# shgaurav1/DVG

Measured on AMD Instinct MI355X. Metric: predicted frames/sec at 64x64, batch 64, 10-in/10-out, higher is better.
Workload: dtype f32

## Files before the change

dvg_amd/csrc/conv_igemm2.hip:

```cpp
#include <cstdlib>
#include <type_traits>

#include "dvg_common.h"

namespace dvg {

constexpr int DVG_GEMM_WGS_PER_CU = DVG_BF16X3 ? 3 : 4;
constexpr int DVG_GEMM128_WGS = DVG_BF16X3 ? 3 : 2;
constexpr int DVG_GEMM128_GT = DVG_BF16X3 ? 2 : 4;
constexpr int DVG_GEMM_GT = 4;
constexpr int DVG_GEMM128_MIN_WGS = 4 * 768;
[[maybe_unused]] constexpr int DVG_GEMM_NT2 = 256;
constexpr int DVG_TILE16_MIN_WGS = 256;

enum { M2_CONV3 = 0, M2_CONV4S2 = 1, M2_CONVT4S2 = 2, M2_GEMM = 3 };

struct Igemm2Params {
    const float* x = nullptr;
    const float* skip = nullptr;
    const float* w = nullptr;
    const float* scale = nullptr;
    const float* shift = nullptr;
    float* y = nullptr;
    float* y_pool = nullptr;
// ... 1007 lines not shown
    const int a_base = (wm * 32 + l31) * LD + hh * 4;
    const int b_base = (wn * 32 + l31) * LDB + (hh ^ ((l31 >> 3) & 1)) * 4;

    f32x16 acc[4];
#pragma unroll
    for (int f = 0; f < 4; ++f)
#pragma unroll
        for (int i = 0; i < 16; ++i) acc[f][i] = 0.f;

    long offx[FIRST ? 1 : ND];
    unsigned okmask = 0;
#pragma unroll
    for (int i = 0; i < ND; ++i) {
        const int hp = (tid + i * 256) >> 2;
        const int yy = yin0 + hp / C::HW, xx = xin0 + hp % C::HW;
        const bool ok = hp < C::HP && (unsigned)yy < (unsigned)p.H && (unsigned)xx < (unsigned)p.W;
        okmask |= ok ? (1u << i) : 0u;
        if constexpr (!FIRST) offx[i] = ok ? (((long)n0 * p.H + yy) * p.W + xx) * p.C1 + (tid & 3) * 4 : 0;
    }
    const int xf = (tid >> 2) & 3, xq = tid & 3;
    const int x_ia = xf == 0 ? 0 : (xf == 2 ? 2 : 1), x_ib = xf == 2 ? 1 : (xf == 3 ? 3 : 2);
    const float x_sg = xf == 1 ? 1.f : -1.f;
    const int x_pix = (tid >> 7) * C::HW + 2 * ((tid >> 4) & 7);
    const int x_da = (x_pix + x_ia) * 16 + xq * 4, x_db = (x_pix + x_ib) * 16 + xq * 4;
    const int x_st = xf * C::PLANE + (tid >> 4) * LD + (xq >> 1) * 4 + (xq & 1) * 2;

    f32x4 fw[FIRST ? 11 : 1];
    f32x4 ra[ND], rb[NLB];
    auto gload_d = [&](int c0) {
        if constexpr (FIRST) {
            const float* w = p.first_w + c0 + (tid & 3) * 4;
#pragma unroll
            for (int tp = 0; tp < 9; ++tp) fw[tp] = *reinterpret_cast<const f32x4*>(w + tp * 64);
            fw[9] = *reinterpret_cast<const f32x4*>(p.first_scale + c0 + (tid & 3) * 4);
            fw[10] = *reinterpret_cast<const f32x4*>(p.first_shift + c0 + (tid & 3) * 4);
        } else {
            const float* src = p.x + c0;
#pragma unroll
            for (int i = 0; i < ND; ++i)
                ra[i] = *reinterpret_cast<const f32x4*>(((okmask >> i) & 1u) ? src + offx[i] : dvg_zero_slot);
        }
    };
    auto store_d = [&]() {
        if constexpr (FIRST) {
#pragma unroll
            for (int i = 0; i < ND; ++i) {
                const int hp = min((tid + i * 256) >> 2, C::HP - 1);
                const float* f = Fp + (hp / C::HW) * C::FP_W + hp % C::HW;
                f32x4 v = {0.f, 0.f, 0.f, 0.f};
#pragma unroll
                for (int tp = 0; tp < 9; ++tp) {
                    const float px = f[(tp / 3) * C::FP_W + tp % 3];
#pragma unroll
                    for (int e = 0; e < 4; ++e) v[e] = fmaf(fw[tp][e], px, v[e]);
                }
                const float okf = (float)((okmask >> i) & 1u);
#pragma unroll
                for (int e = 0; e < 4; ++e) {
                    const float a = v[e] * fw[9][e] + fw[10][e];
                    v[e] = fmaxf(a, a * p.first_slope) * okf;
                }
                ra[i] = v;
            }
        }
#pragma unroll
        for (int i = 0; i < ND; ++i) reinterpret_cast<f32x4*>(Ds)[tid + i * 256] = ra[i];
    };
    auto gload_b = [&](int chunk, int r) {
        const float* tile = p.w + (((size_t)chunk * (p.Cout >> 6) + nb) * 12 + r * 4) * (64 * C::WROW);
#pragma unroll
        for (int j = 0; j < NLB; ++j) rb[j] = reinterpret_cast<const f32x4*>(tile)[tid + j * 256];
    };
    auto store_b = [&]() {
#pragma unroll
        for (int j = 0; j < NLB; ++j) reinterpret_cast<f32x4*>(Bs)[tid + j * 256] = rb[j];
    };
    auto xform_read = [&](u32x2_t (&pa)[NX][3]) {
#pragma unroll
        for (int s = 0; s < NX; ++s) {
            const f32x4 a = *reinterpret_cast<const f32x4*>(&Ds[x_da + s * 2 * C::HW * 16]);
            const f32x4 b = *reinterpret_cast<const f32x4*>(&Ds[x_db + s * 2 * C::HW * 16]);
            f32x4 v;
#pragma unroll
            for (int e = 0; e < 4; ++e) v[e] = fmaf(x_sg, b[e], a[e]);
            unsigned t0, t1, t2;
            bf16x3_split_pair(v[0], v[1], t0, t1, t2);
            pa[s][0][0] = t0; pa[s][1][0] = t1; pa[s][2][0] = t2;
            bf16x3_split_pair(v[2], v[3], t0, t1, t2);
            pa[s][0][1] = t0; pa[s][1][1] = t1; pa[s][2][1] = t2;
        }
    };
    auto xform_store = [&](const u32x2_t (&pa)[NX][3]) {
#pragma unroll
        for (int s = 0; s < NX; ++s)
#pragma unroll
            for (int j = 0; j < 3; ++j) *reinterpret_cast<u32x2_t*>(&As[x_st + s * 16 * LD + j * 8]) = pa[s][j];
    };

    if constexpr (FIRST) {
        const float* fr = p.first_frame + (size_t)n0 * p.H * p.W;
        for (int i = tid; i < C::FP_FLOATS; i += 256) {
            const int yy = yin0 - 1 + i / C::FP_W, xx = xin0 - 1 + i % C::FP_W;
            Fp[i] = ((unsigned)yy < (unsigned)p.H && (unsigned)xx < (unsigned)p.W) ? fr[(size_t)yy * p.W + xx] : 0.f;
        }
        __syncthreads();
    }
    gload_d(0);
    gload_b(0, 0);
    store_d();
    store_b();
    __syncthreads();
    {
        u32x2_t pa[NX][3];
        xform_read(pa);
        xform_store(pa);
    }
    __syncthreads();

    auto stage = [&](const int chunk, auto r_c, auto next_chunk_c, auto has_next_c) __attribute__((always_inline)) {
        constexpr int R = decltype(r_c)::value;
        constexpr bool NEXT_CHUNK = decltype(next_chunk_c)::value, HAS_NEXT = decltype(has_next_c)::value;
        constexpr bool LOAD_D = NEXT_CHUNK && R == 0, STORE_D = NEXT_CHUNK && R == 1, XFORM = NEXT_CHUNK && R == 2;
        if constexpr (LOAD_D) gload_d((chunk + 1) * 16);
        if constexpr (HAS_NEXT) gload_b(R == 2 ? chunk + 1 : chunk, (R + 1) % 3);
        if constexpr (STORE_D) store_d();
        u32x2_t pa[XFORM ? NX : 1][3];
        if constexpr (XFORM) xform_read(pa);

        f32x4 fa[2][3], fb[2][3];
#pragma unroll
        for (int j = 0; j < 3; ++j) {
            fa[0][j] = *reinterpret_cast<const f32x4*>(&As[a_base + R * C::TP * LD + j * 8]);
            fb[0][j] = *reinterpret_cast<const f32x4*>(&Bs[b_base + j * 8]);
        }
#pragma unroll
        for (int tt = 0; tt < 4; ++tt) {
            const int cur = tt & 1, nxt = cur ^ 1;
            if (tt + 1 < 4) {
#pragma unroll
                for (int j = 0; j < 3; ++j) {
                    fa[nxt][j] = *reinterpret_cast<const f32x4*>(&As[a_base + (tt + 1) * C::PLANE + R * C::TP * LD + j * 8]);
                    fb[nxt][j] = *reinterpret_cast<const f32x4*>(&Bs[b_base + (tt + 1) * 64 * LDB + j * 8]);
                }
            }
            if (HAS_NEXT && tt == 3) {
                __syncthreads();
                if constexpr (XFORM) xform_store(pa);
                store_b();
            }
            auto mm = [&](int pa_, int pb_) {
                acc[tt] = __builtin_amdgcn_mfma_f32_32x32x16_bf16(__builtin_bit_cast(bf16x8_t, fa[cur][pa_]),
                                                                  __builtin_bit_cast(bf16x8_t, fb[cur][pb_]), acc[tt], 0, 0, 0);
            };
            mm(2, 0);
            mm(1, 1);
            mm(0, 2);
            mm(1, 0);
            mm(0, 1);
            mm(0, 0);
            constexpr int NREAD = 6, NMFMA = 6;
            constexpr int NVMEM = (LOAD_D ? (FIRST ? 11 : ND) : 0) + (HAS_NEXT ? NLB : 0), VPT = (NVMEM + 2) / 3;
            if (tt == 0) __builtin_amdgcn_sched_group_barrier(0x100, NREAD + (XFORM ? 2 * NX : 0) + (STORE_D && FIRST ? 9 * ND : 0), 0);
            if (tt + 1 < 4) {
#pragma unroll
                for (int r = 0; r < NREAD; ++r) {
                    __builtin_amdgcn_sched_group_barrier(0x100, 1, 0);
                    __builtin_amdgcn_sched_group_barrier(0x008, 1, 0);
                }
                if (VPT > 0) __builtin_amdgcn_sched_group_barrier(0x020, VPT, 0);
            } else if (HAS_NEXT) {
                constexpr int NW = NLB + (XFORM ? 3 * NX : 0);
#pragma unroll
                for (int r = 0; r < NW; ++r) {
                    if (r < NMFMA) __builtin_amdgcn_sched_group_barrier(0x008, 1, 0);
                    __builtin_amdgcn_sched_group_barrier(0x200, 1, 0);
                }
            } else if (!HAS_NEXT) {
                __builtin_amdgcn_sched_group_barrier(0x008, NMFMA, 0);
            }
        }
        if constexpr (HAS_NEXT) __syncthreads();
    };
    using std::integral_constant;
    using T_ = integral_constant<bool, true>;
    using F_ = integral_constant<bool, false>;
    int st = 0;
    auto set_prio = [&]() {
        switch (st++ & 3) {
            case 0: __builtin_amdgcn_s_setprio(3); break;
            case 1: __builtin_amdgcn_s_setprio(2); break;
            case 2: __builtin_amdgcn_s_setprio(1); break;
            default: __builtin_amdgcn_s_setprio(0); break;
        }
    };
    const int nchunks = p.C1 / 16;
    int chunk = 0;
    for (; chunk + 1 < nchunks; ++chunk) {
        set_prio();
        stage(chunk, integral_constant<int, 0>{}, T_{}, T_{});
        set_prio();
        stage(chunk, integral_constant<int, 1>{}, T_{}, T_{});
        set_prio();
        stage(chunk, integral_constant<int, 2>{}, T_{}, T_{});
    }
    set_prio();
    stage(chunk, integral_constant<int, 0>{}, F_{}, T_{});
    set_prio();
    stage(chunk, integral_constant<int, 1>{}, F_{}, T_{});
    set_prio();
    stage(chunk, integral_constant<int, 2>{}, F_{}, F_{});
    __builtin_amdgcn_s_setprio(0);

    const int c = nb0 + wn * 32 + l31;
    const float sc = p.scale ? p.scale[c] : 1.f, sf = p.shift ? p.shift[c] : 0.f;
    const bool want_y = !FIRST || n0 >= p.y_from;
    float* const yb = p.y + (size_t)n0 * p.H * p.W * p.Cout + c;
    float* const pb = p.y_pool ? p.y_pool + (size_t)n0 * (p.H >> 1) * (p.W >> 1) * p.Cout + c : nullptr;
    const float* ab = nullptr;
    if (p.addend) ab = p.addend + (size_t)(addend_image(p.add_map, p.add_B, n0)) * p.H * p.W * p.Cout + c;
    auto epilogue = [&](auto act_c) {
        constexpr int ACT = decltype(act_c)::value;
        float v[2][16];
#pragma unroll
        for (int reg = 0; reg < 16; ++reg) {
            v[0][reg] = (acc[0][reg] + acc[1][reg]) + acc[2][reg];
            v[1][reg] = (acc[1][reg] - acc[2][reg]) - acc[3][reg];
        }
#pragma unroll
        for (int reg = 0; reg < 16; ++reg) {
            const int m = wm * 32 + (reg & 3) + 8 * (reg >> 2) + 4 * hh;
            const int off = ((y0 + (m >> 3)) * p.W + x0 + 2 * (m & 7)) * p.Cout;
#pragma unroll
            for (int e = 0; e < 2; ++e) {
                float u = v[e][reg];
                if (ab != nullptr) u += ab[off + e * p.Cout];
                u = u * sc + sf;
                if constexpr (ACT == DVG_ACT_LRELU) u = u > 0.f ? u : u * p.slope;
                else if constexpr (ACT != DVG_ACT_NONE) u = apply_act(u, p.act, p.slope);
                v[e][reg] = u;
                if (want_y) yb[off + e * p.Cout] = u;
            }
        }
        if (pb != nullptr) {
#pragma unroll
            for (int reg = 0; reg < 16; ++reg) {
                if (((reg >> 2) & 1) == 0) {
                    const int m = wm * 32 + (reg & 3) + 8 * (reg >> 2) + 4 * hh;
                    const float mx = fmaxf(fmaxf(v[0][reg], v[1][reg]), fmaxf(v[0][reg + 4], v[1][reg + 4]));
                    pb[(((y0 + (m >> 3)) >> 1) * (p.W >> 1) + (x0 >> 1) + (m & 7)) * p.Cout] = mx;
                }
            }
        }
    };
    if (p.act == DVG_ACT_LRELU) epilogue(std::integral_constant<int, DVG_ACT_LRELU>{});
    else if (p.act == DVG_ACT_NONE) epilogue(std::integral_constant<int, DVG_ACT_NONE>{});
    else epilogue(std::integral_constant<int, -1>{});
}

template <bool FIRST>
static int launch_wx(Igemm2Params p, hipStream_t stream) {
    using C = CfgWX;
    p.tiles_y = p.H / C::TH;
    p.tiles_x = p.W / C::TW;
    p.tiles_n = p.N;
    p.nblk_n = p.Cout / 64;
    const long tiles = (long)p.tiles_y * p.tiles_x * p.tiles_n;
    p.nb_group = choose_nb_group(tiles, p.nblk_n, 12.0 * p.C1 * 64 * 4, (double)C::TH * C::TW * p.C1 * 4);
    static bool attr_set = false;
    if (!attr_set) {
        hipError_t e = hipFuncSetAttribute(reinterpret_cast<const void*>(&conv3_wx_kernel<FIRST>),
                                           hipFuncAttributeMaxDynamicSharedMemorySize, C::lds_bytes(FIRST));
        if (e != hipSuccess) return fail(DVG_ERR_HIP, "hipFuncSetAttribute: %s", hipGetErrorString(e));
        attr_set = true;
    }
    hipLaunchKernelGGL((conv3_wx_kernel<FIRST>), dim3((unsigned)(tiles * p.nblk_n)), dim3(256), C::lds_bytes(FIRST), stream, p);
    return check_launch("conv3_wx");
}
#endif

__global__ void pack_wx_kernel(const float* __restrict__ src, float* __restrict__ dst, int cout, int cin) {
    const long total = (long)cout * cin * 12 / 2;
    const int nblk = cout >> 6;
    for (long i = blockIdx.x * (long)blockDim.x + threadIdx.x; i < total; i += (long)gridDim.x * blockDim.x) {
        const int k = (int)(i & 7) * 2;
        long r = i >> 3;
        const int co = r % cout; r /= cout;
        const int tap = r % 12;
        const int chunk = r / 12;
        const int row = tap >> 2, f = tap & 3;
        float u[2];
#pragma unroll
        for (int e = 0; e < 2; ++e) {
            const float* g = src + (((long)co * cin + chunk * 16 + k + e) * 3 + row) * 3;
            if (f == 0) u[e] = g[0];
            else if (f == 1) u[e] = ((g[0] + g[1]) + g[2]) * 0.5f;
            else if (f == 2) u[e] = ((g[0] - g[1]) + g[2]) * 0.5f;
            else u[e] = g[2];
        }
        wrow_store_pair(dst, (((size_t)chunk * nblk + (co >> 6)) * 12 + tap) * 64 + (co & 63), co & 63, k, u[0], u[1]);
    }
    wrow_drain();
}

__global__ void pack_k16_kernel(const float* __restrict__ src, float* __restrict__ dst, int cout, int cin, int kh,
                                int kw, int transposed) {
    const long total = (long)cout * cin * kh * kw / 2;
    const int nblk = cout >> 6, taps = kh * kw;
    for (long i = blockIdx.x * (long)blockDim.x + threadIdx.x; i < total; i += (long)gridDim.x * blockDim.x) {
        const int k = (int)(i & 7) * 2;
        long r = i >> 3;
        const int co = r % cout; r /= cout;
        const int t = r % taps;
        const int chunk = r / taps;
        const int ci = chunk * 16 + k, a = t / kw, b = t % kw;
        const long j = transposed ? ((((long)ci * cout + co) * kh + (kh - 1 - a)) * kw + (kw - 1 - b))
                                  : ((((long)co * cin + ci) * kh + a) * kw + b);
        const long j1 = j + (transposed ? (long)cout * kh * kw : (long)kh * kw);
        int slot = t;
        if (transposed && kh == 4 && kw == 4) {
            const int py = a & 1, px = b & 1;
            slot = (py * 2 + px) * 4 + ((2 + py - a) >> 1) * 2 + ((2 + px - b) >> 1);
        } else if (kh == 4 && kw == 4) {
            slot = ((a & 1) * 2 + (b & 1)) * 4 + (a >> 1) * 2 + (b >> 1);
        }
        wrow_store_pair(dst, (((size_t)chunk * nblk + (co >> 6)) * taps + slot) * 64 + (co & 63), co & 63, k, src[j], src[j1]);
    }
    wrow_drain();
}

}

using namespace dvg;

extern "C" int dvg_mfma_mode(void) { return DVG_BF16X3 ? 1 : 0; }
extern "C" int dvg_packed_row_floats(void) { return DVG_WROW; }

extern "C" void dvg_debug_set_clockbuf(void* buf, unsigned records) {
    g_clk = (unsigned long long*)buf;
    g_clk_cap = buf ? records : 0;
}

extern "C" int dvg_pack_conv_weight_k16(const float* w, float* w_packed, int cout, int cin, int kh, int kw,
                                        int transposed, void* stream) {
    DVG_REQUIRE(w && w_packed, DVG_ERR_NULL, "dvg_pack_conv_weight_k16: NULL pointer");
    DVG_REQUIRE(cout > 0 && cout % 64 == 0 && cin > 0 && cin % 16 == 0 && kh > 0 && kw > 0, DVG_ERR_SHAPE,
                "dvg_pack_conv_weight_k16: Cin must be a multiple of 16, Cout of 64");
    const long total = (long)cout * cin * kh * kw / 2;
    long g = (total + 255) / 256;
    if (g > 4096) g = 4096;
    hipLaunchKernelGGL(pack_k16_kernel, dim3((unsigned)g), dim3(256), 0, (hipStream_t)stream, w, w_packed, cout, cin, kh,
                       kw, transposed);
    return check_launch("dvg_pack_conv_weight_k16");
}

extern "C" int dvg_conv_splitk_v2(int mode, int N, int H, int W, int Cin, int Cout) {
    Plan2 pl;
    if (Cin % 16 || Cout % 64 || plan2(&pl, mode, N, H, W, Cin, Cout, true, false)) return -1;
    return pl.splitk;
}

extern "C" int dvg_conv_stats_rows_v2(int mode, int N, int H, int W, int Cin, int Cout, int pool, int with_workspace) {
    Plan2 pl;
    if (plan2(&pl, mode, N, H, W, Cin, Cout, with_workspace != 0, pool != 0)) return -1;
    return pl.stats_rows;
}

static Igemm2Params params2(const float* x, const float* skip, const float* w, const float* scale, const float* shift, float* y,
                            int N, int H, int W, int C1, int C2, int Cout, int act, float slope) {
    Igemm2Params p{};
    p.x = x; p.skip = skip; p.w = w; p.scale = scale; p.shift = shift; p.y = y;
    p.N = N; p.H = H; p.W = W; p.C1 = C1; p.C2 = C2; p.Cout = Cout;
    p.act = act; p.slope = slope;
    return p;
}

static int set_addend(Igemm2Params& p, const char* who, const float* addend, const int* addend_map, int addend_block) {
    p.addend = addend;
    p.add_map = addend ? addend_map : nullptr;
    p.add_B = addend_block;
    DVG_REQUIRE(p.add_map == nullptr || (addend_block > 0 && p.N % addend_block == 0), DVG_ERR_SHAPE,
                "%s: addend_block must divide N", who);
    return DVG_OK;
}

static int checks2(const Igemm2Params& p, const char* who) {
    DVG_REQUIRE(p.x && p.w && p.y, DVG_ERR_NULL, "%s: x/w/y must not be NULL", who);
    DVG_REQUIRE((p.skip != nullptr) == (p.C2 > 0), DVG_ERR_SHAPE, "%s: skip pointer / C2 mismatch", who);
    DVG_REQUIRE(p.N > 0 && p.H > 0 && p.W > 0, DVG_ERR_SHAPE, "%s: empty shape", who);
    DVG_REQUIRE(p.C1 > 0 && p.C1 % 16 == 0 && p.C2 % 16 == 0, DVG_ERR_SHAPE, "%s: C1=%d C2=%d must be multiples of 16",
                who, p.C1, p.C2);
    DVG_REQUIRE(p.Cout > 0 && p.Cout % 64 == 0, DVG_ERR_SHAPE, "%s: Cout=%d must be a multiple of 64", who, p.Cout);
    DVG_REQUIRE(aligned16(p.x) && aligned16(p.w) && aligned16(p.y) && aligned16(p.skip), DVG_ERR_ALIGN,
                "%s: pointers must be 16-byte aligned", who);
    DVG_REQUIRE(p.act >= DVG_ACT_NONE && p.act <= DVG_ACT_SIGMOID, DVG_ERR_SHAPE, "%s: bad act", who);
    return DVG_OK;
}

extern "C" int dvg_conv3x3_bn_act_v2(const float* x, const float* skip, const float* w_k16, const float* scale,
                                     const float* shift, float* y, float* y_pool, float* stats, int N, int H, int W,
                                     int C1, int C2, int Cout, int upsample_x, int act, float slope,
                                     float* workspace, long workspace_floats, const float* addend,
                                     const int* addend_map, int addend_block, void* stream) {
    const char* who = "dvg_conv3x3_bn_act_v2";
    Igemm2Params p = params2(x, skip, w_k16, scale, shift, y, N, H, W, C1, C2, Cout, act, slope);
    p.y_pool = y_pool;
    p.stats = stats;
    p.upsample = upsample_x ? 1 : 0;
    if (int e = set_addend(p, who, addend, addend_map, addend_block)) return e;
    if (int e = checks2(p, who)) return e;
    DVG_REQUIRE(aligned16(addend) && (addend == nullptr || y_pool == nullptr), DVG_ERR_SHAPE,
                "%s: addend must be 16-byte aligned and excludes the pooled output", who);
    DVG_REQUIRE(H % 8 == 0 && W % 8 == 0, DVG_ERR_SHAPE, "%s: H=%d W=%d must be multiples of 8", who, H, W);
    Plan2 pl;
    DVG_REQUIRE(plan2(&pl, M2_CONV3, N, H, W, C1 + C2, Cout, workspace != nullptr, y_pool != nullptr) == 0 && pl.ti == 1,
                DVG_ERR_SHAPE, "%s: no tile for %dx%d", who, H, W);
    return launch_tile<M2_CONV3>(p, pl, who, workspace, workspace_floats, stream);
}

static int first_pair_params(Igemm2Params* out, const char* who, const float* frame, const float* w0, const float* scale0,
                             const float* shift0, const float* w1, const float* scale1, const float* shift1, float* y,
                             float* y_pool, int N, int H, int W, int Cout, int act, float slope, int y_from) {
    DVG_REQUIRE(y_from >= 0 && y_from <= N && (y_from == 0 || y_pool != nullptr) && (y != nullptr || y_from == N), DVG_ERR_SHAPE,
                "%s: y_from=%d needs 0 <= y_from <= N, a pooled output when > 0, y unless == N", who, y_from);
    float* const y_biased = y ? y - (size_t)y_from * H * W * Cout : y_pool;
    Igemm2Params p = params2(frame , nullptr, w1, scale1, shift1, y_biased, N, H, W, 64, 0, Cout,
                             act, slope);
    p.y_pool = y_pool;
    p.first_frame = frame; p.first_w = w0; p.first_scale = scale0; p.first_shift = shift0; p.first_slope = 0.2f;
    p.y_from = y_from;
    *out = p;
    return DVG_OK;
}

extern "C" int dvg_conv3x3_first_pair(const float* frame, const float* w0, const float* scale0, const float* shift0,
                                      const float* w1_k16, const float* scale1, const float* shift1, float* y, float* y_pool,
                                      int N, int H, int W, int Cout, int act, float slope, int y_from, void* stream) {
    const char* who = "dvg_conv3x3_first_pair";
    DVG_REQUIRE(frame && w0 && scale0 && shift0, DVG_ERR_NULL, "%s: NULL pointer", who);
    Igemm2Params p;
    if (int e = first_pair_params(&p, who, frame, w0, scale0, shift0, w1_k16, scale1, shift1, y, y_pool, N, H, W, Cout, act, slope,
                                  y_from))
        return e;
    if (int e = checks2(p, who)) return e;
    DVG_REQUIRE(H % 8 == 0 && W % 16 == 0 && (long)N * (H / 8) * (W / 16) * (Cout / 64) >= 512, DVG_ERR_SHAPE,
                "%s: H %% 8, W %% 16 and >= 512 workgroups needed (N=%d H=%d W=%d Cout=%d)", who, N, H, W, Cout);
    Plan2 pl;
    if (plan2(&pl, M2_CONV3, N, H, W, 64, Cout, false, y_pool != nullptr, true)) return fail(DVG_ERR_SHAPE, "%s: no tile", who);
    return launch2<M2_CONV3, Tile2<1, 8, 16>, true>(p, pl, nullptr, 0, (hipStream_t)stream);
}

extern "C" int dvg_pack_conv_weight_wx(const float* w, float* w_packed, int cout, int cin, void* stream) {
    DVG_REQUIRE(w && w_packed, DVG_ERR_NULL, "dvg_pack_conv_weight_wx: NULL pointer");
    DVG_REQUIRE(cout > 0 && cout % 64 == 0 && cin > 0 && cin % 16 == 0, DVG_ERR_SHAPE,
                "dvg_pack_conv_weight_wx: Cin must be a multiple of 16, Cout of 64");
    DVG_REQUIRE(aligned16(w_packed), DVG_ERR_ALIGN, "dvg_pack_conv_weight_wx: w_packed must be 16-byte aligned");
    const long total = (long)cout * cin * 12 / 2;
    hipLaunchKernelGGL(pack_wx_kernel, dim3(grid_for(total, 256, 4096)), dim3(256), 0, (hipStream_t)stream, w, w_packed, cout, cin);
    return check_launch("dvg_pack_conv_weight_wx");
}

static int checks_wx(const Igemm2Params& p, const char* who) {
    DVG_REQUIRE(p.N > 0 && p.H > 0 && p.W > 0, DVG_ERR_SHAPE, "%s: empty shape", who);
    DVG_REQUIRE(p.C1 > 0 && p.C1 % 16 == 0 && p.C2 == 0 && p.skip == nullptr && !p.upsample, DVG_ERR_SHAPE,
                "%s: Cin=%d must be a multiple of 16; no concat operand, no upsampling", who, p.C1 + p.C2);
    DVG_REQUIRE(p.Cout > 0 && p.Cout % 64 == 0, DVG_ERR_SHAPE, "%s: Cout=%d must be a multiple of 64", who, p.Cout);
    DVG_REQUIRE(p.H % 8 == 0 && p.W % 16 == 0, DVG_ERR_SHAPE, "%s: H=%d must be a multiple of 8, W=%d of 16", who, p.H, p.W);
    DVG_REQUIRE((long)p.H * p.W * p.Cout < (1L << 31), DVG_ERR_SHAPE, "%s: image of %d x %d x %d floats too large", who, p.H, p.W, p.Cout);
    DVG_REQUIRE(aligned16(p.x) && aligned16(p.w) && aligned16(p.y) && aligned16(p.y_pool) && aligned16(p.addend), DVG_ERR_ALIGN,
                "%s: pointers must be 16-byte aligned", who);
    DVG_REQUIRE(p.act >= DVG_ACT_NONE && p.act <= DVG_ACT_SIGMOID, DVG_ERR_SHAPE, "%s: bad act", who);
    DVG_REQUIRE(DVG_BF16X3 != 0, DVG_ERR_SHAPE, "%s: the f32-MFMA build has no WX kernel", who);
    return DVG_OK;
}

extern "C" int dvg_conv3x3_bn_act_wx(const float* x, const float* skip, const float* w_wx, const float* scale,
                                     const float* shift, float* y, float* y_pool, int N, int H, int W, int C1, int C2,
                                     int Cout, int upsample_x, int act, float slope, const float* addend,
                                     const int* addend_map, int addend_block, void* stream) {
    const char* who = "dvg_conv3x3_bn_act_wx";
    DVG_REQUIRE(x && w_wx && y, DVG_ERR_NULL, "%s: x/w/y must not be NULL", who);
    Igemm2Params p = params2(x, skip, w_wx, scale, shift, y, N, H, W, C1, C2, Cout, act, slope);
    p.y_pool = y_pool;
    p.upsample = upsample_x ? 1 : 0;
    if (int e = set_addend(p, who, addend, addend_map, addend_block)) return e;
    DVG_REQUIRE(addend == nullptr || y_pool == nullptr, DVG_ERR_SHAPE, "%s: addend excludes the pooled output", who);
    if (int e = checks_wx(p, who)) return e;
#if DVG_BF16X3
    return launch_wx<false>(p, (hipStream_t)stream);
#else
    return DVG_ERR_SHAPE;
#endif
}

extern "C" int dvg_conv3x3_first_pair_wx(const float* frame, const float* w0, const float* scale0, const float* shift0,
                                         const float* w1_wx, const float* scale1, const float* shift1, float* y, float* y_pool,
                                         int N, int H, int W, int Cout, int act, float slope, int y_from, void* stream) {
    const char* who = "dvg_conv3x3_first_pair_wx";
    DVG_REQUIRE(frame && w0 && scale0 && shift0 && w1_wx, DVG_ERR_NULL, "%s: NULL pointer", who);
    Igemm2Params p;
    if (int e = first_pair_params(&p, who, frame, w0, scale0, shift0, w1_wx, scale1, shift1, y, y_pool, N, H, W, Cout, act, slope,
                                  y_from))
        return e;
    DVG_REQUIRE(aligned16(w0) && aligned16(scale0) && aligned16(shift0) && aligned16(y), DVG_ERR_ALIGN,
                "%s: pointers must be 16-byte aligned", who);
    if (int e = checks_wx(p, who)) return e;
#if DVG_BF16X3
    return launch_wx<true>(p, (hipStream_t)stream);
#else
    return DVG_ERR_SHAPE;
#endif
}

extern "C" int dvg_conv4x4s2_bn_act_v2(const float* x, const float* w_k16, const float* scale, const float* shift,
                                       float* y, float* stats, int N, int H, int W, int Cin, int Cout, int act,
                                       float slope, float* workspace, long workspace_floats, void* stream) {
    const char* who = "dvg_conv4x4s2_bn_act_v2";
    Igemm2Params p = params2(x, nullptr, w_k16, scale, shift, y, N, H, W, Cin, 0, Cout, act, slope);
    p.stats = stats;
    if (int e = checks2(p, who)) return e;
    DVG_REQUIRE(H % 2 == 0 && W % 2 == 0, DVG_ERR_SHAPE, "%s: odd input", who);
    DVG_REQUIRE((long)N * H * W * Cin < (1L << 31), DVG_ERR_SHAPE,
                "%s: input of %d x %d x %d x %d floats too large (32-bit offsets)", who, N, H, W, Cin);
    Plan2 pl;
    DVG_REQUIRE(plan2(&pl, M2_CONV4S2, N, H, W, Cin, Cout, workspace != nullptr, false) == 0, DVG_ERR_SHAPE,
                "%s: unsupported map %dx%d", who, H, W);
    return launch_tile<M2_CONV4S2, T2_444>(p, pl, who, workspace, workspace_floats, stream);
}

extern "C" int dvg_convT4x4s2_bn_act_v2(const float* x, const float* skip, const float* w_k16, const float* scale,
                                        const float* shift, float* y, float* stats, int N, int H, int W, int C1,
                                        int C2, int Cout, int act, float slope, float* workspace, long workspace_floats,
                                        const float* addend, const int* addend_map, int addend_block, void* stream) {
    const char* who = "dvg_convT4x4s2_bn_act_v2";
    Igemm2Params p = params2(x, skip, w_k16, scale, shift, y, N, H, W, C1, C2, Cout, act, slope);
    p.stats = stats;
    if (int e = set_addend(p, who, addend, addend_map, addend_block)) return e;
    if (int e = checks2(p, who)) return e;
    DVG_REQUIRE(aligned16(addend), DVG_ERR_ALIGN, "%s: addend must be 16-byte aligned", who);
    Plan2 pl;
    DVG_REQUIRE(plan2(&pl, M2_CONVT4S2, N, H, W, C1 + C2, Cout, workspace != nullptr, false) == 0, DVG_ERR_SHAPE,
                "%s: unsupported map %dx%d", who, H, W);
    return launch_tile<M2_CONVT4S2, T2_444>(p, pl, who, workspace, workspace_floats, stream);
}

extern "C" int dvg_convT4x4s2_bn_act_proj(const float* x, const float* w_k16, const float* scale, const float* shift,
                                          const float* proj_w, float* proj_out, int T, int N, int H, int W, int C1, int Cout,
                                          int act, float slope, const float* addend, const int* addend_map, int addend_block,
                                          void* stream) {
    const char* who = "dvg_convT4x4s2_bn_act_proj";
    DVG_REQUIRE(x && w_k16 && proj_w && proj_out, DVG_ERR_NULL, "%s: x / w / proj_w / proj_out must not be NULL", who);
    DVG_REQUIRE(N > 0 && H > 0 && W > 0, DVG_ERR_SHAPE, "%s: empty shape", who);
    DVG_REQUIRE(C1 > 0 && C1 % 16 == 0, DVG_ERR_SHAPE, "%s: C1=%d must be a multiple of 16", who, C1);
    DVG_REQUIRE(Cout == 64, DVG_ERR_SHAPE, "%s: Cout=%d must be 64 (one column block holds every channel of a pixel)", who, Cout);
    DVG_REQUIRE(T >= 1 && T <= 48, DVG_ERR_SHAPE, "%s: T=%d must be in 1..48", who, T);
    DVG_REQUIRE(aligned16(x) && aligned16(w_k16) && aligned16(proj_w) && aligned16(addend), DVG_ERR_ALIGN,
                "%s: pointers must be 16-byte aligned", who);
    DVG_REQUIRE(act >= DVG_ACT_NONE && act <= DVG_ACT_SIGMOID, DVG_ERR_SHAPE, "%s: bad act", who);
    Igemm2Params p = params2(x, nullptr, w_k16, scale, shift, nullptr, N, H, W, C1, 0, Cout, act, slope);
    if (int e = set_addend(p, who, addend, addend_map, addend_block)) return e;
    p.proj_w = proj_w;
    p.proj_out = proj_out;
    p.proj_T = T;
    Plan2 pl;
    DVG_REQUIRE(plan2(&pl, M2_CONVT4S2, N, H, W, C1, Cout, false, false, true) == 0 && pl.ti == 1, DVG_ERR_SHAPE,
                "%s: unsupported map %dx%d (multiples of 8 needed)", who, H, W);
    return launch_tile<M2_CONVT4S2, 0, true>(p, pl, who, nullptr, 0, stream);
}

static int gemm_plan(Plan2* pl, int NB, int nb_tile, int H, int W, int Cin, int Cout) {
    if (NB <= 0 || nb_tile < NB || H <= 0 || W <= 0 || Cin <= 0 || Cout <= 0) return -1;
    if (Cin % (16 * DVG_GEMM_GT) || Cout % 64 || H % 8 || W % 8) return -1;
    return plan2(pl, M2_GEMM, NB, H, W, Cin, Cout, false, false, false, nb_tile);
}

static int gemm_batched(const float* x, const float* w_k16, float* y, int NB, int nb_tile, int H, int W, int Cin, int Cout,
                        void* stream) {
    const char* who = "dvg_gemm_batched_k16";
    Igemm2Params p = params2(x, nullptr, w_k16, nullptr, nullptr, y, NB, H, W, Cin, 0, Cout, DVG_ACT_NONE, 0.f);
    if (int e = checks2(p, who)) return e;
    Plan2 pl;
    DVG_REQUIRE(gemm_plan(&pl, NB, nb_tile, H, W, Cin, Cout) == 0, DVG_ERR_SHAPE,
                "%s: Cin=%d must be a multiple of %d, H=%d W=%d multiples of 8 with a tile", who, Cin, 16 * DVG_GEMM_GT, H, W);
    DVG_REQUIRE((long)H * W * Cin < (1L << 31), DVG_ERR_SHAPE, "%s: image of %d x %d x %d floats too large", who, H, W, Cin);
    p.w_image_stride = (long)Cin / 16 * Cout * DVG_WROW;
    return launch_tile<M2_GEMM, T2_NT2>(p, pl, who, nullptr, 0, stream);
}

extern "C" int dvg_gemm_batched_k16(const float* x, const float* w_k16, float* y, int NB, int H, int W, int Cin, int Cout,
                                    void* stream) {
    return gemm_batched(x, w_k16, y, NB, NB, H, W, Cin, Cout, stream);
}

extern "C" int dvg_gemm_batched_k16_as(const float* x, const float* w_k16, float* y, int NB, int NB_as, int H, int W, int Cin,
                                       int Cout, void* stream) {
    DVG_REQUIRE(NB > 0 && NB_as >= NB, DVG_ERR_SHAPE, "dvg_gemm_batched_k16_as: NB=%d, NB_as=%d (NB_as >= NB > 0 needed)", NB, NB_as);
    return gemm_batched(x, w_k16, y, NB, NB_as, H, W, Cin, Cout, stream);
}

extern "C" int dvg_gemm_batched_plan_as(int NB, int NB_as, int H, int W, int Cin, int Cout, int* tile_w, int* nt, int* ni) {
    Plan2 pl;
    if (!tile_w || !nt || !ni || gemm_plan(&pl, NB, NB_as, H, W, Cin, Cout)) return -1;
    *tile_w = pl.tw; *nt = pl.nt; *ni = pl.ni;
    return 0;
}

extern "C" int dvg_gemm_batched_plan(int NB, int H, int W, int Cin, int Cout, int* tile_w, int* nt, int* ni) {
    return dvg_gemm_batched_plan_as(NB, NB, H, W, Cin, Cout, tile_w, nt, ni);
}
```

dvg_amd/fused.py:

```python
from __future__ import annotations

import collections
import contextlib
import functools
import os
import types
import weakref

import torch
import torch.nn as nn

from . import _derived, ops, weights
from ._derived import derived, version_key as _ver
from .ops import ACT_LRELU, ACT_NONE, ACT_SIGMOID, ACT_TANH, MODE_CONV3, MODE_CONV4S2, MODE_CONVT4S2


WINOGRAD = int(os.environ.get("DVG_WINOGRAD", "4"))
if WINOGRAD not in (0, 2, 4):
    raise RuntimeError("DVG_WINOGRAD must be 0, 2 or 4")


_WINO_MIN_C = 64
_WINO_MAX_HW = 32


WINOGRAD_LAYER_OVERRIDE = {}


def winograd_tile(n, c, h, w, cout) -> int:
    if WINOGRAD_LAYER_OVERRIDE:
        forced = WINOGRAD_LAYER_OVERRIDE.get((c, h, cout))
        if forced is not None:
            return forced if (forced == 0 or ops.winograd_ok(n, c, h, w, cout, forced)) else 0
    if WINOGRAD >= 4 and c >= _WINO_MIN_C and h <= _WINO_MAX_HW and w <= _WINO_MAX_HW and ops.winograd_ok(n, c, h, w, cout, 4):
        return 4
    if WINOGRAD >= 2 and c >= 256 and ops.winograd_ok(n, c, h, w, cout, 2) and \
            ((h <= 8 and w <= 8) or (h <= 16 and w <= 16 and cout >= 256)):
        return 2
    return 0


UPCONV_WINOGRAD = True
_UPCONV_WINO_MAX = 16
UPCONV_WINO_LIVE = True


def folded_affine(conv: nn.Module, bn: nn.BatchNorm2d):
    def build():
        with torch.no_grad():
            inv = torch.rsqrt(bn.running_var + bn.eps)
            scale = (bn.weight * inv) if bn.weight is not None else inv
            bias = conv.bias if conv.bias is not None else torch.zeros_like(bn.running_mean)
            shift = (bias - bn.running_mean) * scale
            if bn.bias is not None:
                shift = shift + bn.bias
            return scale.contiguous(), shift.contiguous()

    return derived(bn, "fold", (conv.bias, bn.weight, bn.bias, bn.running_mean, bn.running_var), build)


def _needs_grad(*ts) -> bool:
    return torch.is_grad_enabled() and any(
        t is not None and (t.t if isinstance(t, ops.SharedBlocks) else t).requires_grad for t in ts)


def _no_shared(skip, who):
    if isinstance(skip, ops.SharedBlocks):
        raise RuntimeError(f"{who}: shared skip blocks (time-batched decoder calls) are a training-path operand (autograd)")


def _bias(conv):
    return conv.bias.detach() if conv.bias is not None else None


Block = collections.namedtuple("Block", "raw mode finish cat dgrad")


def _raw_conv3(x, skip, wp, b, *, up=False, stats=False, addend=None):
    return ops.conv3x3(x, skip, wp, None, b, upsample=up, act=ACT_NONE, stats=stats, addend=addend)


def _raw_convT4s2(x, skip, wp, b, *, up=False, stats=False, addend=None):
    if up:
        raise RuntimeError("convT4s2: no fused upsampling")
    return ops.convT4x4s2(x, skip, wp, None, b, act=ACT_NONE, stats=stats, addend=addend)


def _raw_plain(name):
    def raw(x, skip, w, b, *, up=False, stats=False, addend=None):
        if skip is not None or up or addend is not None:
            raise RuntimeError(f"{name}: neither a concat conv nor an upsampling one")
        return getattr(ops, name)(x, w, None, b, act=ACT_NONE, stats=stats)
    return raw


def _dgrad_conv3(du, weight, lo, hi):
    n, c, h, w = du.shape
    m = winograd_tile(n, c, h, w, hi - lo)
    if m:
        return ops.conv3x3_winograd(du, weights.winograd(weight, m, lo, hi, dgrad=True), None, None, act=ACT_NONE)
    return ops.conv3x3(du, None, weights.packed(weight, True, lo, hi, 1), None, None, act=ACT_NONE)


def _dgrad_conv4s2(du, weight, lo, hi):
    return ops.convT4x4s2(du, None, weights.packed(weight, True, lo, hi, 1), None, None, act=ACT_NONE)


def _dgrad_convT4s2(du, weight, lo, hi):
    return ops.conv4x4s2(du, weights.packed(weight, False, lo, hi, 0), None, None, act=ACT_NONE)


BLOCKS = {
    "conv3": Block(_raw_conv3, MODE_CONV3, (0, 3, 3), 1, _dgrad_conv3),
    "conv4s2": Block(_raw_plain("conv4x4s2"), MODE_CONV4S2, (0, 4, 4), 1, _dgrad_conv4s2),
    "convT4s2": Block(_raw_convT4s2, MODE_CONVT4S2, (1, 4, 4), 0, _dgrad_convT4s2),
    "conv3_first": Block(_raw_plain("conv3x3_first"), None, (0, 3, 3), 1, None),
    "conv4s2_first": Block(_raw_plain("conv4x4s2_first"), None, (0, 4, 4), 1, None),
}


def block_weight(kind, weight, lo=None, hi=None):
    blk = BLOCKS[kind]
    return weight if blk.mode is None else weights.packed(weight, bool(blk.finish[0]), lo, hi, blk.cat)


CONV3_WX = True
CONV3_WX_MIN_WGS = 256


def conv3_wx_applies(n, cin, h, w, cout, *modules) -> bool:
    return (CONV3_WX and not torch.is_grad_enabled() and not any(m.training for m in modules)
            and ops.lib().dvg_tile_policy() == 1 and cin == 64 and w >= 64 and ops.wx_ok(n, cin, h, w, cout)
            and ops.wx_workgroups(n, h, w, cout) >= CONV3_WX_MIN_WGS)


def _skip_half(kind, skip, ps, conv=None):
    if kind == "conv3" and conv is not None and not conv.training and not torch.is_grad_enabled():
        n, c, h, w = skip.shape
        ctot = conv.weight.shape[1]
        if winograd_tile(n, c, h, w, conv.weight.shape[0]) == 4:
            return ops.conv3x3_winograd(skip, weights.winograd(conv.weight, 4, ctot - c, ctot), None, None, act=ACT_NONE)
        if conv3_wx_applies(n, c, h, w, conv.weight.shape[0], conv):
            return ops.conv3x3_wx(skip, weights.wx(conv.weight, ctot - c, ctot), None, None, act=ACT_NONE)
    return BLOCKS[kind].raw(skip, None, ps, None)


_scope = types.SimpleNamespace(passes=1, groups=None, trace=None, share=None)


@contextlib.contextmanager
def _scoped(result=None, **fields):
    prev = {k: getattr(_scope, k) for k in fields}
    vars(_scope).update(fields)
    try:
        yield result
    finally:
        vars(_scope).update(prev)


def bn_passes(k: int):
    return _scoped(passes=int(k))


def bn_momentum(bn, passes=None) -> float:
    m = bn.momentum if bn.momentum is not None else 0.1
    return 1.0 - (1.0 - m) ** (_scope.passes if passes is None else passes)


def bn_passes_now() -> int:
    return _scope.passes


_GROUP_STATS_RECOMPUTE = False


def bn_groups(groups: int, passes=(1, 1, 1)):
    return _scoped(groups=(int(groups),) + tuple(int(k) for k in passes) if groups > 1 else None)


def bn_groups_now() -> int:
    return _scope.groups[0] if _scope.groups else 1


def group_stats(st, u):
    g = bn_groups_now()
    if g == 1:
        return st
    if st is not None and getattr(st, "grouped", 0) == g:
        return st
    ti = getattr(st, "tile_images", 0) if st is not None else 0
    if ti and not _GROUP_STATS_RECOMPUTE and st.shape[0] % g == 0 and (u.shape[0] // g) % ti == 0:
        return st
    u2 = u if u.dim() == 2 else u.permute(0, 2, 3, 1).reshape(-1, u.shape[1])
    return ops.channel_stats(u2, g)


def bn_counter(bn):
    return bn.num_batches_tracked if (bn.track_running_stats and bn.num_batches_tracked is not None) else None


def bn_trace():
    trace = types.SimpleNamespace(entries=[])
    return _scoped(trace, trace=trace.entries)


def replay_bn_trace(entries) -> None:
    for bn, stats, count, passes, groups in entries:
        with _scoped(trace=None, groups=groups, passes=passes):
            _train_bn(bn, stats, count, synced=True)


_SYNC_BN = None


def set_sync_bn(dist=None, group=None) -> None:
    global _SYNC_BN
    if dist is None or not dist.is_initialized() or dist.get_world_size(group) <= 1:
        _SYNC_BN = None
    else:
        _SYNC_BN = (dist, group, dist.get_world_size(group))
    ops.set_sync_bn_state(_SYNC_BN)


def sync_bn_world() -> int:
    return _SYNC_BN[2] if _SYNC_BN is not None else 1


def _train_bn(bn: nn.BatchNorm2d, stats, count, save=False, synced=False):
    grouped, passes = _scope.groups, _scope.passes
    g = grouped[0] if grouped else 1
    if _SYNC_BN is not None and not synced:
        stats = ops.sync_partial_rows(stats, g)
        count = count * _SYNC_BN[2]
    if _scope.trace is not None:
        _scope.trace.append((bn, stats, count, passes, grouped))
    if grouped:
        _, p0, p1, p2 = grouped
        if passes != 1 or count % g:
            raise RuntimeError("grouped BatchNorm: bn_passes must be 1 and the groups must divide the batch")
        momentum, passes, momenta = 0.0, p0 + p2 + (g - 2) * p1, tuple(bn_momentum(bn, k) for k in (p0, p1, p2))
    else:
        momentum, momenta = bn_momentum(bn), None
    return ops.bn_finalize(stats, bn.weight.detach() if bn.weight is not None else None,
                           bn.bias.detach() if bn.bias is not None else None,
                           bn.running_mean if bn.track_running_stats else None,
                           bn.running_var if bn.track_running_stats else None, count // g, bn.eps, momentum, save=save,
                           num_batches_tracked=bn_counter(bn), passes=passes, groups=g, group_momenta=momenta)



SKIP_HOIST = os.environ.get("DVG_SKIP_HOIST", "1") != "0"
UPCONV_AS_CONVT = os.environ.get("DVG_UPCONV_AS_CONVT", "1") != "0"
LAST_PROJ_FUSED = True
_skip_seen = {}


_frozen = {}


def clear_skip_hoist_cache():
    _skip_seen.clear()
    _frozen.clear()


_derived.register("skip_hoist", clear_skip_hoist_cache, _skip_seen.values, skip_keyed=(_skip_seen, _frozen))


def declare_frozen_skips(skips) -> None:
    if not SKIP_HOIST:
        return
    for dead in [k for k, e in _frozen.items() if e[0]() is None]:
        del _frozen[dead]
    for s in skips:
        _frozen[id(s)] = (weakref.ref(s), s._version)


def share_skip_halves():
    return _scoped(share={})


def skip_share_scope():
    return _scope.share


def precompute_skip_half(conv, skip, kind: str) -> None:
    if not SKIP_HOIST or skip is None:
        return
    ctot = conv.weight.shape[BLOCKS[kind].cat]
    s = _skip_half(kind, skip, block_weight(kind, conv.weight, ctot - skip.shape[1], ctot), conv)
    _skip_seen[(id(conv), id(skip))] = [weakref.ref(skip), skip._version, _ver(conv.weight), 1, s]


def _hoisted_skip(conv, x, skip, partial_fn, force=False):
    if skip is None or (not SKIP_HOIST and not force):
        return None
    k = (id(conv), id(skip))
    wkey = _ver(conv.weight)
    ent = _skip_seen.get(k)
    if ent is None or ent[0]() is not skip or ent[1] != skip._version or ent[2] != wkey:
        for dead in [kk for kk, e in _skip_seen.items() if e[0]() is None]:
            del _skip_seen[dead]
        if len(_skip_seen) > 64:
            _skip_seen.clear()
        _skip_seen[k] = ent = [weakref.ref(skip), skip._version, wkey, 1, None]
        fz = _frozen.get(id(skip))
        if not force and (fz is None or fz[0]() is not skip or fz[1] != skip._version):
            return None
    else:
        ent[3] += 1
    px, ps = weights.split_packed(conv.weight, x.shape[1], isinstance(conv, nn.ConvTranspose2d))
    if ent[4] is None:
        ent[4] = partial_fn(ps)
    return px, ent[4]


WINOGRAD_CHAIN = os.environ.get("DVG_WINOGRAD_CHAIN", "1") != "0"


_CHAIN_LEVEL = int(os.environ.get("DVG_WINOGRAD_CHAIN", "3"))


def _chain_to(conv_next, n, c, h, w, pool=False):
    if not (WINOGRAD_CHAIN and WINOGRAD >= 4 and conv_next is not None and not conv_next.training
            and isinstance(conv_next, nn.Conv2d) and conv_next.weight.shape[1] == c and tuple(conv_next.kernel_size) == (3, 3)):
        return False
    if pool:
        return (_CHAIN_LEVEL >= 2 and winograd_tile(n, c, h // 2, w // 2, conv_next.weight.shape[0]) == 4
                and ops.winograd_pool_chain_ok(n, c, h, w))
    if h > 16 and _CHAIN_LEVEL < 2:
        return False
    return winograd_tile(n, c, h, w, conv_next.weight.shape[0]) == 4 and ops.winograd_chain_ok(n, c, h, w)


def _from(res, y_from):
    if not y_from:
        return res
    y, yp = res
    return (y[y_from:] if y_from < y.shape[0] else None), yp


def _hoist_ready(conv, skip) -> bool:
    if not SKIP_HOIST or skip is None:
        return False
    ent = _skip_seen.get((id(conv), id(skip)))
    if ent is not None and ent[0]() is skip and ent[1] == skip._version and ent[2] == _ver(conv.weight):
        return True
    fz = _frozen.get(id(skip))
    return fz is not None and fz[0]() is skip and fz[1] == skip._version


def _chain_up_to(next_up, n, c, h, w, stem=False) -> bool:
    if next_up is None or torch.is_grad_enabled():
        return False
    conv_n, bn_n, skip_n = next_up
    if not (WINOGRAD_CHAIN and _CHAIN_LEVEL >= 3 and WINOGRAD >= 4 and UPCONV_WINOGRAD and isinstance(conv_n, nn.Conv2d)
            and tuple(conv_n.kernel_size) == (3, 3) and not conv_n.training and not bn_n.training and skip_n is not None
            and not isinstance(skip_n, ops.SharedBlocks)):
        return False
    if conv_n.weight.shape[1] - skip_n.shape[1] != c or tuple(skip_n.shape) != (n, skip_n.shape[1], 2 * h, 2 * w):
        return False
    return (2 * h <= _UPCONV_WINO_MAX and winograd_tile(n, c, 2 * h, 2 * w, conv_n.weight.shape[0]) == 4
            and ((h, w) == (4, 4) if stem else ops.winograd_up_chain_ok(n, c, h, w)) and _hoist_ready(conv_n, skip_n))


def _hand_over(x, next_conv, next_up, n, c, h, w, pool=False):
    if not isinstance(x, ops.WinoV) and torch.is_grad_enabled():
        return False
    if _chain_to(next_conv, n, c, h, w, pool):
        return True
    return "up" if not pool and _chain_up_to(next_up, n, c, h, w) else False


def _bn_act_train(bn, u, st, *, act, slope=0.2, pool=False):
    n, _, h, w = u.shape
    sc, sh = _train_bn(bn, group_stats(st, u), n * h * w)
    return ops.bn_act_apply(u, sc, sh, act=act, slope=slope, pool=pool, inplace=True)


def _train_block(kind, conv, bn, x, skip=None, *, up=False, act, slope, pool=False):
    u, st = BLOCKS[kind].raw(x, skip, block_weight(kind, conv.weight), _bias(conv), up=up, stats=True)
    return _bn_act_train(bn, u, st, act=act, slope=slope, pool=pool)


def _last_proj_applies(next_last, conv, x) -> bool:
    if not LAST_PROJ_FUSED or next_last is None or torch.is_grad_enabled() or not isinstance(next_last, nn.ConvTranspose2d):
        return False
    w = next_last.weight
    return (conv.weight.shape[0] == 64 and w.shape[0] == 64 and tuple(w.shape[2:]) == (3, 3) and 9 * w.shape[1] <= ops.PROJ_MAX_T
            and tuple(next_last.stride) == (1, 1) and tuple(next_last.padding) == (1, 1) and x.shape[2] % 8 == 0
            and x.shape[3] % 8 == 0)


def _upconv_x_winograd(conv, affine, x, s, live, act, slope, next_conv):
    n, c1, h, w = x.shape if isinstance(x, ops.WinoV) else (x.shape[0], x.shape[1], 2 * x.shape[2], 2 * x.shape[3])
    u = weights.winograd_live(conv.weight, 0, c1) if live else weights.winograd(conv.weight, 4, 0, c1)
    to_v = _hand_over(x, next_conv, None, n, conv.weight.shape[0], h, w)
    return ops.conv3x3_winograd(x, u, *affine, act=act, slope=slope, upsample=True, addend=s, to_v=to_v, live=live)


def _winograd_layer(conv, affine, x, m, act, slope, pool, y_from, next_conv, next_up):
    n, _, h, w = x.shape
    to_v = m == 4 and _hand_over(x, next_conv, next_up, n, conv.weight.shape[0], h, w, pool)
    return ops.conv3x3_winograd(x, weights.winograd(conv.weight, m), *affine, act=act, slope=slope, pool=pool, to_v=to_v,
                                y_from=y_from, up_live=UPCONV_WINO_LIVE and to_v == "up")


def conv3_bn_act(conv, bn, x, skip=None, *, upsample=False, pool=False, act=ACT_LRELU, slope=0.2, next_conv=None, y_from=0,
                 next_up=None, next_last=None):
    if y_from and (not pool or bn.training or _needs_grad(x, skip, conv.weight, bn.weight)):
        raise RuntimeError("conv3_bn_act: y_from is an eval-mode, no-grad option of the pooled form")
    if isinstance(x, ops.WinoV) and x.up:
        hs = None if (bn.training or not upsample or pool) else \
            _hoisted_skip(conv, x, skip, functools.partial(_skip_half, "conv3", skip, conv=conv), force=True)
        if hs is None:
            raise RuntimeError("conv3_bn_act: an upsampled WinoV needs the eval-mode concat conv with its skip half hoisted")
        return _upconv_x_winograd(conv, folded_affine(conv, bn), x, hs[1], x.live, act, slope, next_conv)
    if isinstance(x, ops.WinoV):
        if bn.training or skip is not None or upsample:
            raise RuntimeError("conv3_bn_act: a WinoV input needs an eval-mode plain 3x3 layer")
        if winograd_tile(*x.shape, conv.weight.shape[0]) != 4:
            raise RuntimeError("conv3_bn_act: WinoV handed to a layer that is not F(4x4,3x3)")
        return _winograd_layer(conv, folded_affine(conv, bn), x, 4, act, slope, pool, y_from, next_conv, next_up)
    if _needs_grad(x, skip, conv.weight, bn.weight):
        from .autograd import conv_block_autograd
        return conv_block_autograd("conv3", conv, bn, x, skip, upsample=upsample, pool=pool, act=act, slope=slope)
    _no_shared(skip, "conv3_bn_act")
    if not bn.training:
        sc, sh = folded_affine(conv, bn)
        if not pool:
            hs = _hoisted_skip(conv, x, skip, functools.partial(_skip_half, "conv3", skip, conv=conv))
            if hs is not None:
                if upsample and UPCONV_WINOGRAD:
                    n, c1, hx, wx = x.shape
                    if 2 * hx <= _UPCONV_WINO_MAX and winograd_tile(n, c1, 2 * hx, 2 * wx, conv.weight.shape[0]) == 4:
                        live = UPCONV_WINO_LIVE and not torch.is_grad_enabled()
                        return _upconv_x_winograd(conv, (sc, sh), x, hs[1], live, act, slope, next_conv)
                if upsample and UPCONV_AS_CONVT:
                    k4 = weights.k4_packed(conv.weight, x.shape[1])
                    if _last_proj_applies(next_last, conv, x):
                        w_last = next_last.weight
                        d = ops.convT4x4s2_proj(x, k4, sc, sh, ops._last_wmat_cached(w_last, 0, 64, 9 * w_last.shape[1]), act=act,
                                                slope=slope, addend=hs[1])
                        return ops.LastProj(d, (x.shape[0], 64, 2 * x.shape[2], 2 * x.shape[3]), w_last)
                    return ops.convT4x4s2(x, None, k4, sc, sh, act=act, slope=slope, addend=hs[1])
                return ops.conv3x3(x, None, hs[0], sc, sh, upsample=upsample, act=act, slope=slope, addend=hs[1])
        if skip is None and not upsample:
            m = winograd_tile(*x.shape, conv.weight.shape[0])
            if m:
                return _winograd_layer(conv, (sc, sh), x, m, act, slope, pool, y_from, next_conv, next_up)
            if conv3_wx_applies(*x.shape, conv.weight.shape[0], conv, bn):
                return _from(ops.conv3x3_wx(x, weights.wx(conv.weight), sc, sh, act=act, slope=slope, pool=pool), y_from)
        return _from(ops.conv3x3(x, skip, weights.packed(conv.weight), sc, sh, upsample=upsample, act=act, slope=slope,
                                 pool=pool), y_from)
    return _train_block("conv3", conv, bn, x, skip, up=upsample, act=act, slope=slope, pool=pool)


def conv3_first_bn_act(conv, bn, x_nchw, *, act=ACT_LRELU, slope=0.2):
    if _needs_grad(x_nchw, conv.weight, bn.weight):
        from .autograd import conv_block_autograd
        return conv_block_autograd("conv3_first", conv, bn, x_nchw, None, act=act, slope=slope)
    if not bn.training:
        sc, sh = folded_affine(conv, bn)
        return ops.conv3x3_first(x_nchw, conv.weight, sc, sh, act=act, slope=slope)
    return _train_block("conv3_first", conv, bn, x_nchw, act=act, slope=slope)


FIRST_PAIR = True


def first_pair_applies(conv0, bn0, conv1, bn1, x_nchw) -> bool:
    if not FIRST_PAIR or bn0.training or bn1.training or _needs_grad(x_nchw, conv0.weight, bn0.weight, conv1.weight, bn1.weight):
        return False
    n, nc, h, w = x_nchw.shape
    return conv0.out_channels == 64 and conv1.in_channels == 64 and ops.first_pair_ok(n, nc, h, w, conv1.out_channels)


def conv3_first_pair(conv0, bn0, conv1, bn1, x_nchw, *, pool=False, slope=0.2, y_from=0):
    sc0, sh0 = folded_affine(conv0, bn0)
    sc1, sh1 = folded_affine(conv1, bn1)
    n, _, h, w = x_nchw.shape
    if conv3_wx_applies(n, 64, h, w, conv1.out_channels, conv0, bn0, conv1, bn1):
        return ops.conv3x3_first_pair_wx(x_nchw, weights.first_pair_taps(conv0.weight), sc0, sh0, weights.wx(conv1.weight), sc1, sh1,
                                         slope=slope, pool=pool, y_from=y_from)
    return ops.conv3x3_first_pair(x_nchw, weights.first_pair_taps(conv0.weight), sc0, sh0, weights.packed(conv1.weight), sc1, sh1,
                                  slope=slope, pool=pool, y_from=y_from)


def conv4s2_bn_act(conv, bn, x, *, act=ACT_LRELU, slope=0.2):
    if _needs_grad(x, conv.weight, bn.weight):
        from .autograd import conv_block_autograd
        return conv_block_autograd("conv4s2", conv, bn, x, None, act=act, slope=slope)
    if not bn.training:
        sc, sh = folded_affine(conv, bn)
        return ops.conv4x4s2(x, weights.packed(conv.weight), sc, sh, act=act, slope=slope)
    return _train_block("conv4s2", conv, bn, x, act=act, slope=slope)


def conv4s2_first_bn_act(conv, bn, x_nchw, *, act=ACT_LRELU, slope=0.2):
    if _needs_grad(x_nchw, conv.weight, bn.weight):
        from .autograd import conv_block_autograd
        return conv_block_autograd("conv4s2_first", conv, bn, x_nchw, None, act=act, slope=slope)
    if not bn.training:
        sc, sh = folded_affine(conv, bn)
        return ops.conv4x4s2_first(x_nchw, conv.weight, sc, sh, act=act, slope=slope)
    return _train_block("conv4s2_first", conv, bn, x_nchw, act=act, slope=slope)


def convT4s2_bn_act(conv, bn, x, skip=None, *, act=ACT_LRELU, slope=0.2):
    if _needs_grad(x, skip, conv.weight, bn.weight):
        from .autograd import conv_block_autograd
        return conv_block_autograd("convT4s2", conv, bn, x, skip, act=act, slope=slope)
    _no_shared(skip, "convT4s2_bn_act")
    if not bn.training:
        sc, sh = folded_affine(conv, bn)
        hs = _hoisted_skip(conv, x, skip, functools.partial(_skip_half, "convT4s2", skip))
        if hs is not None:
            return ops.convT4x4s2(x, None, hs[0], sc, sh, act=act, slope=slope, addend=hs[1])
        return ops.convT4x4s2(x, skip, weights.packed(conv.weight, True), sc, sh, act=act, slope=slope)
    return _train_block("convT4s2", conv, bn, x, skip, act=act, slope=slope)


def head_bn_tanh(conv, bn, x):
    if _needs_grad(x, conv.weight, bn.weight):
        from .autograd import dense_block_autograd
        return dense_block_autograd("head", conv, bn, x, act=ACT_TANH)
    n, c, h, w = x.shape
    if (h, w) != tuple(conv.kernel_size):
        raise RuntimeError(f"encoder head expects a {conv.kernel_size} map, got {(h, w)}")
    gw = weights.gemm_operand(conv.weight, "head")
    a = x.permute(0, 2, 3, 1).reshape(n, h * w * c)
    k = a.shape[1]
    splitk = max(1, min(64, k // 128))
    if not bn.training:
        sc, sh = folded_affine(conv, bn)
        return ops.gemm_nt(a, gw, sc, sh, act=ACT_TANH, splitk=splitk)
    u = ops.gemm_nt(a, gw, None, _bias(conv), act=ACT_NONE, splitk=splitk)
    u4 = u.view(n, 1, 1, u.shape[1]).permute(0, 3, 1, 2)
    return _bn_act_train(bn, u4, ops.channel_stats(u, bn_groups_now()), act=ACT_TANH).reshape(n, u.shape[1])


def stem_bn_act(conv, bn, vec, *, act=ACT_LRELU, slope=0.2, next_up=None):
    if _needs_grad(vec, conv.weight, bn.weight):
        from .autograd import dense_block_autograd
        return dense_block_autograd("stem", conv, bn, vec, act=act, slope=slope)
    dim, cout, kh, kw = conv.weight.shape
    vec = vec.reshape(-1, dim)
    n = vec.shape[0]
    gw = weights.gemm_operand(conv.weight, "stem")
    if not bn.training:
        sc, sh = folded_affine(conv, bn)
        wt = weights.gemm_operand(conv.weight, "stem_t")
        if wt is not None and (kh, kw) == (4, 4) and cout % 16 == 0 and _chain_up_to(next_up, n, cout, 4, 4, stem=True):
            return ops.stem_up_winograd_input(vec, wt, dim, sc, sh, cout, act=act, slope=slope, live=UPCONV_WINO_LIVE)
    out = ops.nhwc_empty(n, cout, kh, kw, vec.device)
    out2d = out.permute(0, 2, 3, 1).reshape(n, kh * kw * cout)
    if not bn.training:
        if wt is not None:
            ops.stem_gemm(vec, wt, dim, sc, sh, out2d, period=cout, act=act, slope=slope)
        else:
            ops.gemm_nt(vec, gw, sc, sh, act=act, slope=slope, period=cout, out=out2d)
        return out
    ops.gemm_nt(vec, gw, None, _bias(conv), act=ACT_NONE, period=cout, out=out2d)
    return _bn_act_train(bn, out, ops.channel_stats(out2d.view(n * kh * kw, cout), bn_groups_now()), act=act, slope=slope)


def convT3_last(conv, x, *, act=ACT_SIGMOID):
    if isinstance(x, ops.LastProj):
        return ops.convT_last_two_step(x, None, conv.weight, _bias(conv), conv.weight.shape[1], 3, act=act)
    if _needs_grad(x, conv.weight):
        from .autograd import last_layer_autograd
        return last_layer_autograd("convT3", conv, x, None, act=act)
    return ops.convT_last_two_step(x, None, conv.weight, _bias(conv), conv.weight.shape[1], 3, act=act)


def convT4s2_last(conv, x, skip, *, act=ACT_TANH):
    if _needs_grad(x, skip, conv.weight):
        from .autograd import last_layer_autograd
        return last_layer_autograd("convT4s2", conv, x, skip, act=act)
    _no_shared(skip, "convT4s2_last")
    return ops.convT_last_two_step(x, skip, conv.weight, _bias(conv), conv.weight.shape[1], 4, act=act)
```

dvg_amd/ops/__init__.py:

```python
from ._core import (
    ACT_NONE, ACT_LRELU, ACT_TANH, ACT_SIGMOID, MODE_CONV3, MODE_CONV4S2, MODE_CONVT4S2, _stream, KernelTimer,
    set_timer, _run, _p, _dev_f32, nhwc_empty, is_nhwc, to_nhwc, to_nchw, tile_policy,
)
from .conv import (
    pack_conv_weight, pack_convT_weight, packed_row_floats, pack_igemm_weight, _wp_dims, unpack_conv_weight,
    pack_wx_weight, wx_ok, wx_workgroups, conv3x3_wx,
    unpack_convT_weight, _splitk_ws, _SPLITK_WS, evict_captured_workspaces, _stats_buf, _tile_images, SharedBlocks,
    _MAP_CACHE, shared_map, group_sum, _check_addend, conv3x3, CONV4S2_MAX_FLOATS, conv4x4s2, convT4x4s2,
    PROJ_MAX_T, convT4x4s2_proj,
)
from .winograd import (
    winograd_weight, winograd_ok, WinoV, LIVE_POSITIONS, winograd_chain_ok, winograd_up_chain_ok, winograd_pool_chain_ok,
    conv3x3_winograd, stem_up_winograd_input,
)
from .edge import (
    conv3x3_first, first_pair_ok, conv3x3_first_pair, conv3x3_first_pair_wx, convT3x3_last, conv4x4s2_first, convT4x4s2_last, pixel_proj,
    _SKIP_PROJ_CACHE, clear_skip_proj_cache, _cached_skip_proj, _last_wmat, _last_wmat_cached,
    precompute_skip_proj, LastProj, convT_last_two_step, eval_frames, eval_frames_finn, pairwise_frame_mse, moving_mnist_compose, clip_gather, clip_gather_aug, CLIP_MAX_SHIFT,
    mnist_scale_u8, moving_mnist_compose_u8, frame_mosaic, QUANT_TRUNC, QUANT_NEAREST,
    MOSAIC_BLACK, MOSAIC_RED, MOSAIC_GREEN, MOSAIC_SEL_NONE, MOSAIC_SEL_BEST, MOSAIC_SEL_PICK, MOSAIC_CELL_INTS,
)
from .dense import (
    gemm_nt, lstm_cell, lstm_cell_pre, lstm_cell_bwd, lstm_cell_x, stem_gemm, transpose2d, colsum, GEMM_TN_MAX_ROWS,
    gemm_tn, lstm_gates_bwd, gru_cell, gru_cell_pre, rnn_cell, gru_gates_bwd,
)
from .norm import (
    channel_stats, set_sync_bn_state, sync_bn_state, sync_partial_rows, bn_finalize, bn_act_apply, bn_act_bwd,
)
from .gp import (
    gp_predict, gp_var_norms, gp_trigger_step, gp_trigger_replay, gp_trigger_select, gp_trigger_rows, TRIGGER_NEVER, gp_elbo, gp_elbo_bwd,
    sum_steps, gp_step_group, gp_train_bwd, GP_KERNELS, gp_kernel_code, gp_score, gp_score_slots, gp_score_accumulators,
)
from .backward import (
    _LOSS_W, frame_losses, FRAME_LOSS_KINDS, frame_losses_ext, frame_ssim_loss, mse_sum_grad, conv_wgrad_partial, conv_wgrad_partial_multi, winograd_wgrad_ok,
    winograd_wgrad_partial_multi, wgrad_finish, k4_to_w3, conv_wgrad, wgrad_thin, act_bwd, upsample2x_bwd, adam_step, adam_step_guarded,
    optim_step, ADAM, ADAMW, SGD, RMSPROP, NESTEROV,
)
from .guard import grad_sumsq_blocks, grad_sumsq, grad_guard_finish
from .ema import ema_update_blocks, ema_update
from .lr_schedule import LR_KINDS, lr_schedule_tick
from .validate import val_accumulators, val_accumulate
from .resample import resample_u8, resample_band
from .._lib import check, lib


def __getattr__(name):
    if name == "GP_SCORE_SLOTS":
        from . import gp
        return gp.__getattr__(name)
    raise AttributeError(f"module {__name__!r} has no attribute {name!r}")
```

dvg_amd/ops/conv.py:

```python
from __future__ import annotations

import torch

from .._derived import register
from .._lib import check, lib
from ._core import ACT_LRELU, MODE_CONV3, MODE_CONV4S2, MODE_CONVT4S2, _dev_f32, _p, _run, _stream, is_nhwc, nhwc_empty


def pack_conv_weight(w: torch.Tensor) -> torch.Tensor:
    _dev_f32(w, "pack_conv_weight")
    w = w.detach().contiguous()
    co, ci, kh, kw = w.shape
    out = torch.empty((kh * kw, co, ci), device=w.device, dtype=torch.float32)
    check(lib().dvg_pack_conv_weight(_p(w), _p(out), co, ci, kh, kw, _stream()), "pack_conv_weight")
    return out


def pack_convT_weight(w: torch.Tensor) -> torch.Tensor:
    _dev_f32(w, "pack_convT_weight")
    w = w.detach().contiguous()
    ci, co, kh, kw = w.shape
    out = torch.empty((kh * kw, co, ci), device=w.device, dtype=torch.float32)
    check(lib().dvg_pack_convT_weight(_p(w), _p(out), ci, co, kh, kw, _stream()), "pack_convT_weight")
    return out


def packed_row_floats() -> int:
    return int(lib().dvg_packed_row_floats())


def pack_igemm_weight(w: torch.Tensor, transposed: bool = False) -> torch.Tensor:
    _dev_f32(w, "pack_igemm_weight")
    w = w.detach().contiguous()
    if transposed:
        ci, co, kh, kw = w.shape
    else:
        co, ci, kh, kw = w.shape
    out = torch.empty((ci // 16, kh * kw, co, packed_row_floats()), device=w.device, dtype=torch.float32)
    check(lib().dvg_pack_conv_weight_k16(_p(w), _p(out), co, ci, kh, kw, int(transposed), _stream()), "pack_k16")
    return out


def _wp_dims(wp: torch.Tensor):
    if wp.dim() != 4 or wp.shape[3] != packed_row_floats():
        raise RuntimeError(f"packed igemm weight must be [Cin/16][taps][Cout][{packed_row_floats()}], got {tuple(wp.shape)}")
    return wp.shape[1], wp.shape[2], wp.shape[0] * 16


def unpack_conv_weight(wp: torch.Tensor, kh: int, kw: int) -> torch.Tensor:
    t, co, ci = wp.shape
    out = torch.empty((co, ci, kh, kw), device=wp.device, dtype=torch.float32)
    check(lib().dvg_unpack_conv_weight(_p(wp.contiguous()), _p(out), co, ci, kh, kw, _stream()), "unpack_conv_weight")
    return out


def unpack_convT_weight(wp: torch.Tensor, kh: int, kw: int) -> torch.Tensor:
    t, co, ci = wp.shape
    out = torch.empty((ci, co, kh, kw), device=wp.device, dtype=torch.float32)
    check(lib().dvg_unpack_convT_weight(_p(wp.contiguous()), _p(out), ci, co, kh, kw, _stream()),
          "unpack_convT_weight")
    return out


def _splitk_ws(mode, n, h, w, cin, cout, out_numel, device, s=None):
    if s is None:
        s = lib().dvg_conv_splitk_v2(mode, n, h, w, cin, cout)
    if s <= 1:
        return None
    stream = torch.cuda.current_stream(device).cuda_stream
    key = (device.index if device.index is not None else torch.cuda.current_device(), stream, s * out_numel,
           lib().dvg_stream_capture_id(stream))
    ws = _SPLITK_WS.get(key)
    if ws is None:
        if len(_SPLITK_WS) > 256:
            _SPLITK_WS.clear()
        ws = _SPLITK_WS[key] = torch.empty(s * out_numel, device=device, dtype=torch.float32)
    return ws


_SPLITK_WS = {}
register("splitk_ws", _SPLITK_WS.clear, _SPLITK_WS.values)


def evict_captured_workspaces() -> None:
    for k in [k for k in _SPLITK_WS if k[-1] != 0]:
        del _SPLITK_WS[k]


def _stats_buf(rows: int, cout: int, device, tile_images: int = 0):
    if rows <= 0:
        raise RuntimeError("unsupported shape for fused BN statistics")
    st = torch.empty((rows, 2, cout), device=device, dtype=torch.float32)
    st.tile_images = tile_images
    return st


def _tile_images(mode, h, w, s):
    return 0 if s > 1 else 4 if ((h // 2, w // 2) if mode == MODE_CONV4S2 else (h, w)) == (4, 4) else 1


def _igemm_buffers(mode, n, h, w, cin, cout, y, pool, stats):
    s = lib().dvg_conv_splitk_v2(mode, n, h, w, cin, cout)
    ws = _splitk_ws(mode, n, h, w, cin, cout, y.numel(), y.device, s)
    if not stats:
        return ws, None
    rows = lib().dvg_conv_stats_rows_v2(mode, n, h, w, cin, cout, int(pool), int(ws is not None))
    return ws, _stats_buf(rows, cout, y.device, _tile_images(mode, h, w, s))


class SharedBlocks:
    __slots__ = ("t", "block", "map_dev", "map_host")

    def __init__(self, t, block, map_dev, map_host):
        self.t, self.block, self.map_dev, self.map_host = t, int(block), map_dev, tuple(map_host)

    @property
    def blocks(self):
        return self.t.shape[0] // self.block

    @property
    def groups(self):
        return len(self.map_host)

    def like(self, t):
        return SharedBlocks(t, self.block, self.map_dev, self.map_host)


_MAP_CACHE = {}
register("group_maps", _MAP_CACHE.clear, _MAP_CACHE.values)


def shared_map(map_host, device):
    key = (tuple(map_host), str(device))
    m = _MAP_CACHE.get(key)
    if m is None:
        if torch.cuda.is_current_stream_capturing():
            raise RuntimeError("shared_map: a new group map cannot be created while a hipGraph is being captured")
        m = _MAP_CACHE[key] = torch.tensor(list(map_host), dtype=torch.int32, device=device)
    return m


def group_sum(src, shared: "SharedBlocks"):
    _dev_f32(src, "group_sum")
    g, blk = shared.groups, shared.block
    if src.shape[0] != g * blk:
        raise RuntimeError(f"group_sum: {src.shape[0]} images are not {g} groups of {blk}")
    per_image = src.numel() // src.shape[0]
    if src.stride(0) != per_image:
        src = src.contiguous()
    dst = torch.empty_strided((shared.blocks * blk,) + tuple(src.shape[1:]), src.stride(), device=src.device,
                              dtype=torch.float32)
    elems = src.numel() // g
    check(lib().dvg_group_sum(_p(src), _p(shared.map_dev), _p(dst), g, shared.blocks, elems, _stream()), "group_sum")
    return dst


def _check_addend(addend, y, excluded):
    if addend is None:
        return None, None, 0
    if excluded:
        raise RuntimeError("addend excludes the pooled output")
    if isinstance(addend, SharedBlocks):
        t = addend.t
        _dev_f32(t, "addend")
        if (tuple(t.shape[1:]) != tuple(y.shape[1:]) or t.stride() != y.stride() or
                y.shape[0] != addend.groups * addend.block):
            raise RuntimeError(f"shared addend {tuple(t.shape)} x {addend.groups} groups does not match {tuple(y.shape)}")
        return t, addend.map_dev, addend.block
    _dev_f32(addend, "addend")
    if tuple(addend.shape) != tuple(y.shape) or addend.stride() != y.stride():
        raise RuntimeError(f"addend {tuple(addend.shape)} must match the output {tuple(y.shape)} (NHWC in memory)")
    return addend, None, 0


def conv3x3(x, skip, wp, scale, shift, *, upsample=False, act=ACT_LRELU, slope=0.2, pool=False, stats=False,
            addend=None):
    _dev_f32(x, "conv3x3.x")
    assert is_nhwc(x), "conv3x3: x must be NHWC in memory"
    n, c1, hx, wx = x.shape
    h, w = (hx * 2, wx * 2) if upsample else (hx, wx)
    c2 = 0
    if skip is not None:
        _dev_f32(skip, "conv3x3.skip")
        assert is_nhwc(skip), "conv3x3: skip must be NHWC in memory"
        c2 = skip.shape[1]
        if tuple(skip.shape) != (n, c2, h, w):
            raise RuntimeError(f"conv3x3: skip shape {tuple(skip.shape)} does not match {(n, c2, h, w)}")
    taps, cout, cin = _wp_dims(wp)
    if taps != 9 or cin != c1 + c2:
        raise RuntimeError(f"conv3x3: packed weight {tuple(wp.shape)} does not match Cin={c1 + c2}")
    y = nhwc_empty(n, cout, h, w, x.device)
    yp = nhwc_empty(n, cout, h // 2, w // 2, x.device) if pool else None
    addend, amap, ablk = _check_addend(addend, y, pool)
    ws, st = _igemm_buffers(MODE_CONV3, n, h, w, cin, cout, y, pool, stats)
    fl, by = 2.0 * n * h * w * cout * 9 * cin, 4.0 * (x.numel() + (skip.numel() if c2 else 0) + n * h * w * cout +
                                                      wp.numel())
    _run("conv3x3_igemm", fl, by, lib().dvg_conv3x3_bn_act_v2, _p(x), _p(skip), _p(wp), _p(scale), _p(shift), _p(y),
         _p(yp), _p(st), n, h, w, c1, c2, cout, int(upsample), act, slope, _p(ws), 0 if ws is None else ws.numel(),
         _p(addend), _p(amap), ablk, _stream())
    out = (y, yp) if pool else y
    return (out, st) if stats else out


def pack_wx_weight(w: torch.Tensor) -> torch.Tensor:
    _dev_f32(w, "pack_wx_weight")
    w = w.detach().contiguous()
    co, ci, kh, kw = w.shape
    if (kh, kw) != (3, 3):
        raise RuntimeError(f"pack_wx_weight: a 3x3 kernel is needed, got {kh}x{kw}")
    out = torch.empty((ci // 16, 12, co, packed_row_floats()), device=w.device, dtype=torch.float32)
    check(lib().dvg_pack_conv_weight_wx(_p(w), _p(out), co, ci, _stream()), "pack_wx")
    return out


def wx_ok(n, cin, h, w, cout) -> bool:
    return cin % 16 == 0 and cout % 64 == 0 and h % 8 == 0 and w % 16 == 0 and lib().dvg_mfma_mode() == 1


def wx_workgroups(n, h, w, cout) -> int:
    return n * (h // 8) * (w // 16) * (cout // 64)


def conv3x3_wx(x, wp, scale, shift, *, act=ACT_LRELU, slope=0.2, pool=False, addend=None):
    _dev_f32(x, "conv3x3_wx.x")
    assert is_nhwc(x), "conv3x3_wx: x must be NHWC in memory"
    n, c1, h, w = x.shape
    taps, cout, cin = _wp_dims(wp)
    if taps != 12 or cin != c1:
        raise RuntimeError(f"conv3x3_wx: packed weight {tuple(wp.shape)} does not match Cin={c1}")
    y = nhwc_empty(n, cout, h, w, x.device)
    yp = nhwc_empty(n, cout, h // 2, w // 2, x.device) if pool else None
    addend, amap, ablk = _check_addend(addend, y, pool)
    alg = 2.0 * n * h * w * cout * 9 * cin
    by = 4.0 * (x.numel() + n * h * w * cout + wp.numel())
    _run("conv3x3_igemm", alg * 12 / 18, by, lib().dvg_conv3x3_bn_act_wx, _p(x), None, _p(wp), _p(scale), _p(shift), _p(y),
         _p(yp), n, h, w, c1, 0, cout, 0, act, slope, _p(addend), _p(amap), ablk, _stream(), alg_flops=alg)
    return (y, yp) if pool else y


CONV4S2_MAX_FLOATS = 1 << 31


def conv4x4s2(x, wp, scale, shift, *, act=ACT_LRELU, slope=0.2, stats=False):
    _dev_f32(x, "conv4x4s2.x")
    assert is_nhwc(x)
    n, cin, h, w = x.shape
    taps, cout, cin_w = _wp_dims(wp)
    if taps != 16 or cin_w != cin:
        raise RuntimeError(f"conv4x4s2: packed weight {tuple(wp.shape)} does not match Cin={cin}")
    y = nhwc_empty(n, cout, h // 2, w // 2, x.device)
    if x.numel() >= CONV4S2_MAX_FLOATS:
        per = (CONV4S2_MAX_FLOATS - 1) // (cin * h * w)
        per -= per % 8
        if per <= 0:
            raise RuntimeError(f"conv4x4s2: one image of {cin} x {h} x {w} exceeds the kernel's 32-bit offsets")
        runs = -(-n // per)
        per = min(per, -(-(-(-n // runs)) // 8) * 8)
        sts = []
        for lo in range(0, n, per):
            r = conv4x4s2(x[lo:lo + per], wp, scale, shift, act=act, slope=slope, stats=stats)
            y[lo:lo + per].copy_(r[0] if stats else r)
            if stats:
                sts.append(r[1])
        if not stats:
            return y
        st = torch.cat(sts)
        ti = {t.tile_images for t in sts}
        st.tile_images = ti.pop() if len(ti) == 1 else 0
        return y, st
    ws, st = _igemm_buffers(MODE_CONV4S2, n, h, w, cin, cout, y, False, stats)
    fl, by = 2.0 * n * (h // 2) * (w // 2) * cout * 16 * cin, 4.0 * (x.numel() + y.numel() + wp.numel())
    _run("conv4x4s2_igemm", fl, by, lib().dvg_conv4x4s2_bn_act_v2, _p(x), _p(wp), _p(scale), _p(shift), _p(y), _p(st),
         n, h, w, cin, cout, act, slope, _p(ws), 0 if ws is None else ws.numel(), _stream())
    return (y, st) if stats else y


def convT4x4s2(x, skip, wp, scale, shift, *, act=ACT_LRELU, slope=0.2, stats=False, addend=None):
    _dev_f32(x, "convT4x4s2.x")
    assert is_nhwc(x)
    n, c1, h, w = x.shape
    c2 = 0
    if skip is not None:
        assert is_nhwc(skip)
        c2 = skip.shape[1]
        if tuple(skip.shape) != (n, c2, h, w):
            raise RuntimeError("convT4x4s2: skip shape mismatch")
    taps, cout, cin = _wp_dims(wp)
    if taps != 16 or cin != c1 + c2:
        raise RuntimeError(f"convT4x4s2: packed weight {tuple(wp.shape)} does not match Cin={c1 + c2}")
    y = nhwc_empty(n, cout, 2 * h, 2 * w, x.device)
    addend, amap, ablk = _check_addend(addend, y, False)
    ws, st = _igemm_buffers(MODE_CONVT4S2, n, h, w, cin, cout, y, False, stats)
    fl = 2.0 * n * h * w * cout * 16 * cin
    by = 4.0 * (x.numel() + (skip.numel() if c2 else 0) + y.numel() + wp.numel())
    _run("convT4x4s2_igemm", fl, by, lib().dvg_convT4x4s2_bn_act_v2, _p(x), _p(skip), _p(wp), _p(scale), _p(shift),
         _p(y), _p(st), n, h, w, c1, c2, cout, act, slope, _p(ws), 0 if ws is None else ws.numel(), _p(addend),
         _p(amap), ablk, _stream())
    return (y, st) if stats else y


PROJ_MAX_T = 48


def convT4x4s2_proj(x, wp, scale, shift, wm, *, act=ACT_LRELU, slope=0.2, addend=None):
    _dev_f32(x, "convT4x4s2_proj.x")
    _dev_f32(wm, "convT4x4s2_proj.wm")
    assert is_nhwc(x)
    n, c1, h, w = x.shape
    taps, cout, cin = _wp_dims(wp)
    if taps != 16 or cin != c1:
        raise RuntimeError(f"convT4x4s2_proj: packed weight {tuple(wp.shape)} does not match Cin={c1}")
    t = wm.shape[0]
    if cout != 64 or tuple(wm.shape) != (t, 64) or not wm.is_contiguous() or not 1 <= t <= PROJ_MAX_T or h % 8 or w % 8:
        raise RuntimeError(f"convT4x4s2_proj: needs Cout = 64, wm (T <= {PROJ_MAX_T}, 64) and a map of multiples of 8; got Cout="
                           f"{cout}, wm {tuple(wm.shape)}, x {tuple(x.shape)}")
    amap, ablk = None, 0
    if addend is not None:
        if isinstance(addend, SharedBlocks):
            if n != addend.groups * addend.block:
                raise RuntimeError("convT4x4s2_proj: shared addend does not match the batch")
            amap, ablk, addend = addend.map_dev, addend.block, addend.t
        elif addend.shape[0] != n:
            raise RuntimeError("convT4x4s2_proj: addend does not match the batch")
        _dev_f32(addend, "convT4x4s2_proj.addend")
        if tuple(addend.shape[1:]) != (64, 2 * h, 2 * w) or not is_nhwc(addend):
            raise RuntimeError(f"convT4x4s2_proj: addend {tuple(addend.shape)} must be NHWC (.,64,{2 * h},{2 * w})")
    d = torch.empty((n * 4 * h * w, t), device=x.device, dtype=torch.float32)
    fl = 2.0 * n * h * w * cout * 16 * cin + 2.0 * n * 4 * h * w * cout * t
    by = 4.0 * (x.numel() + wp.numel() + wm.numel() + (n * 4 * h * w * cout if addend is not None else 0) + d.numel())
    _run("convT4x4s2_igemm", fl, by, lib().dvg_convT4x4s2_bn_act_proj, _p(x), _p(wp), _p(scale), _p(shift), _p(wm), _p(d), t,
         n, h, w, c1, cout, act, slope, _p(addend), _p(amap), ablk, _stream())
    return d
```

dvg_amd/ops/edge.py:

```python
from __future__ import annotations

import numpy as np
import torch

from .._derived import derived, register
from .._lib import CONSTANTS, check, lib
from ._core import ACT_LRELU, ACT_SIGMOID, ACT_TANH, _dev_f32, _p, _run, _stream, is_nhwc, nhwc_empty
from .conv import SharedBlocks, _stats_buf, _wp_dims


def conv3x3_first(x_nchw, w, scale, shift, *, act=ACT_LRELU, slope=0.2, stats=False):
    _dev_f32(x_nchw, "conv3x3_first.x")
    x = x_nchw if x_nchw.is_contiguous() else x_nchw.contiguous()
    n, nc, h, wd = x.shape
    w = w.detach()
    cout = w.shape[0]
    if tuple(w.shape) != (cout, nc, 3, 3) or not w.is_contiguous():
        raise RuntimeError("conv3x3_first: weight must be contiguous (Cout,nc,3,3)")
    y = nhwc_empty(n, cout, h, wd, x.device)
    st = _stats_buf(lib().dvg_conv_first_stats_rows(3, n, h, wd), cout, x.device, 1) if stats else None
    _run("conv3x3_first", 2.0 * n * h * wd * cout * 9 * nc, 4.0 * (x.numel() + n * h * wd * cout),
         lib().dvg_conv3x3_first, _p(x), _p(w), _p(scale), _p(shift), _p(y), _p(st), n, h, wd, nc, cout, act, slope,
         _stream())
    return (y, st) if stats else y


def first_pair_ok(n, nc, h, w, cout) -> bool:
    return nc == 1 and h % 8 == 0 and w % 16 == 0 and cout % 64 == 0 and n * (h // 8) * (w // 16) * (cout // 64) >= 512


def _first_pair(wx, x_nchw, w0, scale0, shift0, w1, scale1, shift1, act, slope, pool, y_from):
    name, wname = ("conv3x3_first_pair_wx", "wx1") if wx else ("conv3x3_first_pair", "wp1")
    _dev_f32(x_nchw, name + ".x")
    x = x_nchw if x_nchw.is_contiguous() else x_nchw.contiguous()
    n, nc, h, wd = x.shape
    taps, cout, cin = _wp_dims(w1)
    w0 = w0.detach()
    ok = h % 8 == 0 and wd % 16 == 0 if wx else first_pair_ok(n, nc, h, wd, cout)
    if nc != 1 or tuple(w0.shape) != (9, 64) or not w0.is_contiguous() or (taps, cin) != (12 if wx else 9, 64) or not ok:
        raise RuntimeError(f"{name}: unsupported shapes x {tuple(x.shape)} w0 {tuple(w0.shape)} {wname} {tuple(w1.shape)}")
    if not 0 <= y_from <= n or (y_from and not pool):
        raise RuntimeError(f"{name}: y_from needs the pooled output and 0 <= y_from <= N")
    y = nhwc_empty(n - y_from, cout, h, wd, x.device) if y_from < n else None
    yp = nhwc_empty(n, cout, h // 2, wd // 2, x.device) if pool else None
    alg = 2.0 * n * h * wd * (64 * 9 + cout * 9 * 64)
    flops = 2.0 * n * h * wd * (64 * 9 + cout * 6 * 64) if wx else alg
    _run("conv3x3_igemm", flops, 4.0 * (x.numel() + (0 if y is None else y.numel()) + (0 if yp is None else yp.numel()) + w1.numel()),
         lib().dvg_conv3x3_first_pair_wx if wx else lib().dvg_conv3x3_first_pair, _p(x), _p(w0), _p(scale0), _p(shift0), _p(w1),
         _p(scale1), _p(shift1), _p(y), _p(yp), n, h, wd, cout, act, slope, y_from, _stream(), alg_flops=alg)
    return (y, yp) if pool else y


def conv3x3_first_pair(x_nchw, w0, scale0, shift0, wp1, scale1, shift1, *, act=ACT_LRELU, slope=0.2, pool=False, y_from=0):
    return _first_pair(False, x_nchw, w0, scale0, shift0, wp1, scale1, shift1, act, slope, pool, y_from)


def conv3x3_first_pair_wx(x_nchw, w0, scale0, shift0, wx1, scale1, shift1, *, act=ACT_LRELU, slope=0.2, pool=False, y_from=0):
    return _first_pair(True, x_nchw, w0, scale0, shift0, wx1, scale1, shift1, act, slope, pool, y_from)


def convT3x3_last(x, w, bias, nc, *, act=ACT_SIGMOID):
    _dev_f32(x, "convT3x3_last.x")
    assert is_nhwc(x)
    n, cin, h, wd = x.shape
    w = w.detach()
    if tuple(w.shape) != (cin, nc, 3, 3) or not w.is_contiguous():
        raise RuntimeError("convT3x3_last: weight must be contiguous (Cin,nc,3,3)")
    y = torch.empty((n, nc, h, wd), device=x.device, dtype=torch.float32)
    _run("convT3x3_last", 2.0 * n * h * wd * cin * 9 * nc, 4.0 * (x.numel() + y.numel()),
         lib().dvg_convT3x3_last, _p(x), _p(w), _p(bias), _p(y), n, h, wd, cin, nc, act, _stream())
    return y


def conv4x4s2_first(x_nchw, w, scale, shift, *, act=ACT_LRELU, slope=0.2, stats=False):
    _dev_f32(x_nchw, "conv4x4s2_first.x")
    x = x_nchw if x_nchw.is_contiguous() else x_nchw.contiguous()
    n, nc, h, wd = x.shape
    w = w.detach()
    cout = w.shape[0]
    if tuple(w.shape) != (cout, nc, 4, 4) or not w.is_contiguous():
        raise RuntimeError("conv4x4s2_first: weight must be contiguous (Cout,nc,4,4)")
    y = nhwc_empty(n, cout, h // 2, wd // 2, x.device)
    st = _stats_buf(lib().dvg_conv_first_stats_rows(4, n, h, wd), cout, x.device, 1) if stats else None
    _run("conv4x4s2_first", 2.0 * n * (h // 2) * (wd // 2) * cout * 16 * nc, 4.0 * (x.numel() + y.numel()),
         lib().dvg_conv4x4s2_first, _p(x), _p(w), _p(scale), _p(shift), _p(y), _p(st), n, h, wd, nc, cout, act, slope,
         _stream())
    return (y, st) if stats else y


def convT4x4s2_last(x, skip, w, bias, nc, *, act=ACT_TANH):
    _dev_f32(x, "convT4x4s2_last.x")
    assert is_nhwc(x)
    n, c1, h, wd = x.shape
    c2 = 0
    if skip is not None:
        assert is_nhwc(skip)
        c2 = skip.shape[1]
    w = w.detach()
    if tuple(w.shape) != (c1 + c2, nc, 4, 4) or not w.is_contiguous():
        raise RuntimeError("convT4x4s2_last: weight must be contiguous (Cin,nc,4,4)")
    y = torch.empty((n, nc, 2 * h, 2 * wd), device=x.device, dtype=torch.float32)
    _run("convT4x4s2_last", 2.0 * n * h * wd * (c1 + c2) * 16 * nc,
         4.0 * (x.numel() + (skip.numel() if c2 else 0) + y.numel()), lib().dvg_convT4x4s2_last, _p(x), _p(skip),
         _p(w), _p(bias), _p(y), n, h, wd, c1, c2, nc, act, _stream())
    return y


def pixel_proj(x, wm):
    assert is_nhwc(x)
    n, c, h, wd = x.shape
    t = wm.shape[0]
    d = torch.empty((n * h * wd, t), device=x.device, dtype=torch.float32)
    _run("pixel_proj", 2.0 * n * h * wd * c * t, 4.0 * (x.numel() + d.numel()), lib().dvg_pixel_proj, _p(x), _p(wm),
         _p(d), n * h * wd, c, t, _stream())
    return d


_SKIP_PROJ_CACHE = {}


def clear_skip_proj_cache():
    _SKIP_PROJ_CACHE.clear()


register("skip_proj", clear_skip_proj_cache, _SKIP_PROJ_CACHE.values, skip_keyed=(_SKIP_PROJ_CACHE,))


def _cached_skip_proj(skip, wm_fn, w):
    import weakref
    key = id(skip)
    ent = _SKIP_PROJ_CACHE.get(key)
    if ent is not None and ent[0]() is skip and ent[1] == skip._version and ent[2] == id(w) and ent[3] == w._version:
        return ent[4]
    d2 = pixel_proj(skip, wm_fn())
    if len(_SKIP_PROJ_CACHE) > 8:
        _SKIP_PROJ_CACHE.clear()
    _SKIP_PROJ_CACHE[key] = (weakref.ref(skip), skip._version, id(w), w._version, d2)
    return d2


def _last_wmat(wpart, t):
    return wpart.permute(2, 3, 1, 0).reshape(t, wpart.shape[0]).contiguous()


def _last_wmat_cached(w, lo, hi, t):
    return derived(w, ("wmat", lo, hi), (w,), lambda: _last_wmat(w.detach()[lo:hi], t))


def precompute_skip_proj(skip, w, ks: int) -> None:
    wdet = w.detach()
    c1 = wdet.shape[0] - skip.shape[1]
    t = ks * ks * wdet.shape[1]
    _cached_skip_proj(skip, lambda: _last_wmat_cached(w, c1, wdet.shape[0], t), w)


class LastProj:

    def __init__(self, d, shape, w):
        self.d, self.shape, self.w = d, tuple(shape), w


def convT_last_two_step(x, skip, w, bias, nc, ks, *, act):
    wdet = w.detach()
    t = ks * ks * nc
    if isinstance(x, LastProj):
        if x.w is not w or tuple(x.d.shape) != (x.shape[0] * x.shape[2] * x.shape[3], t):
            raise RuntimeError("convT_last_two_step: the projection handed over was made for another last layer")
        n, c1, h, wd = x.shape
        d1 = x.d
    else:
        assert is_nhwc(x)
        n, c1, h, wd = x.shape
        d1 = pixel_proj(x, _last_wmat_cached(w, 0, c1, t))
    d2 = None
    d2_map, d2_blk = None, 0
    if isinstance(skip, SharedBlocks):
        d2 = pixel_proj(skip.t, _last_wmat_cached(w, c1, wdet.shape[0], t))
        d2_map, d2_blk = skip.map_dev, skip.block
        if n != skip.groups * skip.block:
            raise RuntimeError("convT_last_two_step: shared skip does not match the batch")
    elif skip is not None:
        d2 = _cached_skip_proj(skip, lambda: _last_wmat_cached(w, c1, wdet.shape[0], t), w)
    s = 2 if ks == 4 else 1
    y = torch.empty((n, nc, s * h, s * wd), device=d1.device, dtype=torch.float32)
    _run("convT_gather", 0.0, 4.0 * (d1.numel() * (2 if skip is not None else 1) + y.numel()), lib().dvg_convT_gather,
         _p(d1), _p(d2), _p(bias), _p(y), ks, n, h, wd, nc, act, _p(d2_map), d2_blk, _stream())
    return y


def eval_frames(gt, pred):
    _dev_f32(gt, "eval_frames.gt")
    _dev_f32(pred, "eval_frames.pred")
    if gt.shape != pred.shape or gt.dim() != 4:
        raise RuntimeError(f"eval_frames: shapes {tuple(gt.shape)} vs {tuple(pred.shape)}")
    gt = gt if gt.is_contiguous() else gt.contiguous()
    pred = pred if pred.is_contiguous() else pred.contiguous()
    b, c, h, w = gt.shape
    out = torch.empty((2, b, c), device=gt.device, dtype=torch.float32)
    _run("eval_frames", 0.0, 8.0 * gt.numel(), lib().dvg_eval_frames, _p(gt), _p(pred), _p(out[0]), _p(out[1]), b * c, h,
         w, _stream())
    return out[0].mean(1), out[1].mean(1)


def eval_frames_finn(gt, pred):
    _dev_f32(gt, "eval_frames_finn.gt")
    _dev_f32(pred, "eval_frames_finn.pred")
    if gt.shape != pred.shape or gt.dim() not in (4, 5):
        raise RuntimeError(f"eval_frames_finn: shapes {tuple(gt.shape)} vs {tuple(pred.shape)}")
    gt = gt if gt.is_contiguous() else gt.contiguous()
    pred = pred if pred.is_contiguous() else pred.contiguous()
    lead, (c, h, w) = tuple(gt.shape[:-3]), gt.shape[-3:]
    n = gt.numel() // (c * h * w)
    out = torch.empty((2, n, c), device=gt.device, dtype=torch.float32)
    mse = torch.empty(n, device=gt.device, dtype=torch.float32)
    _run("eval_frames_finn", 0.0, 8.0 * gt.numel(), lib().dvg_eval_frames_finn, _p(gt), _p(pred), _p(out[0]), _p(out[1]),
         _p(mse), n, c, h, w, _stream())
    if c == 1:
        return out[0].view(lead), out[1].view(lead), mse.view(lead)
    return out[0].mean(1).view(lead), out[1].mean(1).view(lead), mse.view(lead)


def pairwise_frame_mse(samples, lo=None, hi=None):
    _dev_f32(samples, "pairwise_frame_mse.samples")
    if samples.dim() != 6 or samples.numel() == 0 or not samples.is_contiguous():
        raise RuntimeError(f"pairwise_frame_mse: samples {tuple(samples.shape)} must be a contiguous non-empty (S,T,B,C,H,W) tensor")
    s, t, b = samples.shape[:3]
    d = samples[0, 0, 0].numel()
    lo, hi = 0 if lo is None else int(lo), t if hi is None else int(hi)
    if not 0 <= lo < hi <= t:
        raise RuntimeError(f"pairwise_frame_mse: step range [{lo}, {hi}) of {t} steps")
    if d >= 1 << 31 or (hi - lo) * b >= 1 << 31:
        raise RuntimeError(f"pairwise_frame_mse: {hi - lo}x{b} frames of {d} floats exceed the kernel's 32-bit counts")
    out = torch.empty((hi - lo, b, s, s), device=samples.device, dtype=torch.float32)
    n = (hi - lo) * b
    _run("pairwise_frame_mse", 3.0 * n * d * (s * (s - 1) // 2), 4.0 * n * d * s + 4.0 * out.numel(),
         lib().dvg_pairwise_frame_mse, _p(samples[0, lo]), _p(out), s, t * b * d, n, d, d, _stream())
    return out


QUANT_TRUNC, QUANT_NEAREST = CONSTANTS["QUANT_TRUNC"], CONSTANTS["QUANT_NEAREST"]
MOSAIC_BLACK, MOSAIC_RED, MOSAIC_GREEN = (CONSTANTS["MOSAIC_" + k] for k in ("BLACK", "RED", "GREEN"))
MOSAIC_SEL_NONE, MOSAIC_SEL_BEST, MOSAIC_SEL_PICK = (CONSTANTS["MOSAIC_SEL_" + k] for k in ("NONE", "BEST", "PICK"))
MOSAIC_CELL_INTS = CONSTANTS["MOSAIC_CELL_INTS"]


def frame_mosaic(sources, cells, *, nc, H, W, F, R, Cc, cell_h, cell_w, pad_y=0, pad_x=0, oy=0, ox=0, best=None,
                 picks=None, labels=None, quant=QUANT_TRUNC):
    srcs = list(sources) + [None] * (3 - len(sources))
    if len(srcs) != 3:
        raise RuntimeError("frame_mosaic: at most three sources")
    dev, counts = None, []
    for i, s in enumerate(srcs):
        if s is None:
            counts.append(0)
            continue
        _dev_f32(s, f"frame_mosaic.sources[{i}]")
        if not s.is_contiguous() or s.numel() == 0 or s.numel() % (nc * H * W):
            raise RuntimeError(f"frame_mosaic: source {i} {tuple(s.shape)} is not a contiguous run of {nc}x{H}x{W} images")
        counts.append(s.numel() // (nc * H * W))
        dev = s.device
    if dev is None:
        raise RuntimeError("frame_mosaic: no source")

    def aux(t, dtype, dim, name):
        if t is None:
            return
        if not t.is_cuda or t.dtype != dtype or t.dim() != dim or not t.is_contiguous() or t.numel() == 0:
            raise RuntimeError(f"frame_mosaic: {name} must be a contiguous {dim}-D {dtype} device tensor")
    best, picks = (None if t is None else t.contiguous() for t in (best, picks))
    aux(best, torch.int64, 1, "best")
    aux(picks, torch.int32, 2, "picks")
    aux(labels, torch.uint8, 3, "labels")
    if not cells.is_cuda or cells.dtype != torch.int32 or not cells.is_contiguous() or \
            cells.numel() != F * R * Cc * MOSAIC_CELL_INTS:
        raise RuntimeError(f"frame_mosaic: cells must be a contiguous int32 device tensor of {F}x{R}x{Cc}x{MOSAIC_CELL_INTS}")
    gh, gw = R * cell_h + (R - 1) * pad_y, Cc * cell_w + (Cc - 1) * pad_x
    out = torch.empty((F, gh, gw, 3), device=dev, dtype=torch.uint8)
    read = 4.0 * nc * H * W * F * R * Cc
    _run("frame_mosaic", 0.0, read + out.numel(), lib().dvg_frame_mosaic, _p(srcs[0]), counts[0], _p(srcs[1]), counts[1],
         _p(srcs[2]), counts[2], nc, H, W, _p(cells), F, R, Cc, cell_h, cell_w, pad_y, pad_x, oy, ox, _p(best),
         0 if best is None else best.shape[0], _p(picks), 0 if picks is None else picks.shape[0],
         0 if picks is None else picks.shape[1], _p(labels), *((0, 0, 0) if labels is None else labels.shape), quant,
         _p(out), _stream())
    return out


def moving_mnist_compose(sprites, ids, pos, seq_len, image_size):
    _dev_f32(sprites, "moving_mnist_compose.sprites")
    if ids.dtype != torch.int32 or pos.dtype != torch.int32 or not ids.is_cuda or not pos.is_cuda:
        raise RuntimeError("moving_mnist_compose: ids / pos must be int32 device tensors")
    ids, pos, sprites = ids.contiguous(), pos.contiguous(), sprites.contiguous()
    b, nd = ids.shape
    if tuple(pos.shape) != (b, nd, seq_len, 2):
        raise RuntimeError(f"moving_mnist_compose: pos shape {tuple(pos.shape)}")
    out = torch.empty((seq_len, b, 1, image_size, image_size), device=sprites.device, dtype=torch.float32)
    check(lib().dvg_moving_mnist_compose(_p(sprites), _p(ids), _p(pos), _p(out), sprites.shape[0], seq_len, b, nd,
                                         image_size, sprites.shape[1], _stream()), "dvg_moving_mnist_compose")
    return out


def clip_gather(pool, first, T, C):
    if not pool.is_cuda or pool.dtype != torch.uint8 or pool.dim() != 4 or not pool.is_contiguous():
        raise RuntimeError("clip_gather: pool must be a contiguous (n_frames,H,W,pool_c) uint8 GPU tensor - no CPU fallback")
    n, h, w, pc = pool.shape
    if not (isinstance(first, torch.Tensor) and first.is_cuda):
        first = torch.as_tensor(first)
        if first.dtype != torch.int64 or first.dim() != 1 or first.numel() == 0:
            raise RuntimeError("clip_gather: first must be a non-empty 1-D int64 sequence")
        if T < 1 or int(first.min()) < 0 or int(first.max()) + T > n:
            raise RuntimeError(f"clip_gather: clips of {T} frames at [{int(first.min())}, {int(first.max())}] leave the "
                               f"pool of {n} frames")
        first = first.to(pool.device)
    if first.dtype != torch.int64 or first.dim() != 1 or not first.is_contiguous() or first.device != pool.device:
        raise RuntimeError("clip_gather: first must be a contiguous 1-D int64 tensor on the pool's device")
    b = first.shape[0]
    out = torch.empty((max(T, 0), b, C, h, w), device=pool.device, dtype=torch.float32)
    _run("clip_gather", 0.0, float(T * b * h * w * pc) + 4.0 * out.numel(), lib().dvg_clip_gather_u8, _p(pool), _p(first),
         _p(out), n, T, b, C, h, w, pc, _stream())
    return out


CLIP_MAX_SHIFT = 16


def clip_gather_aug(pool, first, geom, photo, T, C):
    if not pool.is_cuda or pool.dtype != torch.uint8 or pool.dim() != 4 or not pool.is_contiguous():
        raise RuntimeError("clip_gather_aug: pool must be a contiguous (n_frames,H,W,pool_c) uint8 GPU tensor - no CPU fallback")
    n, h, w, pc = pool.shape

    def on_device(t):
        return isinstance(t, torch.Tensor) and t.is_cuda

    def host_array(t):
        return np.ascontiguousarray(t.numpy() if isinstance(t, torch.Tensor) else t)
    host = {}
    if not on_device(first):
        f = host_array(first)
        if f.dtype != np.int64 or f.ndim != 1 or f.size == 0:
            raise RuntimeError("clip_gather_aug: first must be a non-empty 1-D int64 sequence")
        if T < 1 or int(f.min()) < 0 or int(f.max()) + T > n:
            raise RuntimeError(f"clip_gather_aug: clips of {T} frames at [{int(f.min())}, {int(f.max())}] leave the pool of "
                               f"{n} frames")
        host["first"] = f
    if not on_device(geom):
        g = host_array(geom)
        if g.dtype != np.int32 or g.ndim != 2 or g.shape[1] != 4 or g.size == 0:
            raise RuntimeError("clip_gather_aug: geom must be a non-empty (B,4) int32 array [hflip, reverse, dy, dx]")
        if int(g[:, 2:].min()) < -CLIP_MAX_SHIFT or int(g[:, 2:].max()) > CLIP_MAX_SHIFT:
            raise RuntimeError(f"clip_gather_aug: a shift (dy, dx) beyond +-{CLIP_MAX_SHIFT} pixels")
        host["geom"] = g
    if not on_device(photo):
        ph = host_array(photo)
        if ph.dtype != np.float32 or ph.ndim != 2 or ph.shape[1] != 2 or ph.size == 0:
            raise RuntimeError("clip_gather_aug: photo must be a non-empty (B,2) float32 array [gain, bias]")
        if not np.isfinite(ph).all():
            raise RuntimeError("clip_gather_aug: gain / bias must be finite")
        host["photo"] = ph
    if len(host) == 3:
        a, b_ = host["first"].nbytes, host["first"].nbytes + host["geom"].nbytes
        buf = np.empty(b_ + host["photo"].nbytes, np.uint8)
        buf[:a], buf[a:b_], buf[b_:] = (host[k].reshape(-1).view(np.uint8) for k in ("first", "geom", "photo"))
# ... 65 lines not shown
```

dvg_amd/weights.py:

```python
from __future__ import annotations

import torch

from . import ops
from ._derived import derived


def _span(weight, lo, hi, dim):
    return (None, None, None) if lo is None or (lo == 0 and hi == weight.shape[dim]) else (lo, hi, dim)


def _sliced(weight, lo, hi, dim):
    w = weight.detach()
    if lo is not None:
        w = w[lo:hi] if dim == 0 else w[:, lo:hi]
    return w.contiguous()


def packed(weight, transposed=False, lo=None, hi=None, dim=0):
    lo, hi, dim = _span(weight, lo, hi, dim)
    return derived(weight, ("wp", transposed, lo, hi, dim), (weight,),
                   lambda: ops.pack_igemm_weight(_sliced(weight, lo, hi, dim), transposed))


def wx(weight, lo=None, hi=None):
    lo, hi, dim = _span(weight, lo, hi, 1)
    return derived(weight, ("wx", lo, hi), (weight,), lambda: ops.pack_wx_weight(_sliced(weight, lo, hi, dim)))


def split_packed(weight, c1: int, transposed=False):
    dim = 0 if transposed else 1
    return packed(weight, transposed, 0, c1, dim), packed(weight, transposed, c1, weight.shape[dim], dim)


def winograd(weight, m, lo=None, hi=None, dgrad=False):
    lo, hi, _ = _span(weight, lo, hi, 1)

    def build():
        w = weight.detach()
        if lo is not None:
            w = w[:, lo:hi]
        if dgrad:
            w = w.transpose(0, 1).flip(2, 3)
        return ops.winograd_weight(w.contiguous(), m)

    return derived(weight, ("wino", m, lo, hi, dgrad), (weight,), build)


def winograd_live(weight, lo=None, hi=None):
    lo, hi, _ = _span(weight, lo, hi, 1)

    def build():
        u = winograd(weight, 4, lo, hi)
        return u.index_select(0, torch.tensor(ops.LIVE_POSITIONS, device=u.device))

    return derived(weight, ("wino_live", lo, hi), (weight,), build)


def k4_weight(weight, c1: int) -> torch.Tensor:
    w = weight.detach()[:, :c1]
    k4 = torch.zeros((w.shape[0], c1, 4, 4), device=w.device, dtype=torch.float32)
    for ty in range(3):
        for tx in range(3):
            k4[:, :, 2 - ty:4 - ty, 2 - tx:4 - tx] += w[:, :, ty:ty + 1, tx:tx + 1]
    return k4.permute(1, 0, 2, 3).contiguous()


def k4_packed(weight, c1: int, adjoint=False):
    def build():
        k4 = derived(weight, ("k4", c1), (weight,), lambda: k4_weight(weight, c1))
        return ops.pack_igemm_weight(k4, transposed=not adjoint)

    return derived(weight, ("k4p", c1, adjoint), (weight,), build)


def transposed(weight):
    return derived(weight, "T", (weight,), lambda: ops.transpose2d(weight.detach()))


def gemm_operand(weight, kind: str):
    def build():
        if kind.endswith("_T"):
            return ops.transpose2d(gemm_operand(weight, kind[:-2]))
        w = weight.detach()
        if kind == "head":
            n, c, kh, kw = w.shape
            return w.permute(0, 2, 3, 1).reshape(n, kh * kw * c).contiguous()
        k, c, kh, kw = w.shape
        if kind == "stem":
            return w.permute(2, 3, 1, 0).reshape(kh * kw * c, k).contiguous()
        gw = None
        if k <= 128 and (kh * kw * c) % 32 == 0:
            gw = torch.zeros((96 if k <= 96 else 128, kh * kw * c), device=w.device, dtype=torch.float32)
            gw[:k] = w.permute(0, 2, 3, 1).reshape(k, kh * kw * c)
        return gw

    if kind not in ("head", "stem", "stem_t", "head_T", "stem_T"):
        raise RuntimeError(kind)
    return derived(weight, ("gw", kind), (weight,), build)


def first_pair_taps(weight):
    return derived(weight, "w_t9x64", (weight,), lambda: weight.detach().reshape(64, 9).t().contiguous())
```

include/dvg_hip.h:

```cpp
#ifndef DVG_HIP_H
#define DVG_HIP_H

#include <stddef.h>
#include <stdint.h>

#ifdef __cplusplus
extern "C" {
#endif

#define DVG_OK 0
#define DVG_ERR_SHAPE 1
#define DVG_ERR_NULL 2
#define DVG_ERR_HIP 3
#define DVG_ERR_ALIGN 4
#define DVG_ACT_NONE 0
#define DVG_ACT_LRELU 1
#define DVG_ACT_TANH 2
#define DVG_ACT_SIGMOID 3
int dvg_abi_version(void);
const char* dvg_last_error(void);
long dvg_stream_capture_id(void* stream);
int dvg_pack_conv_weight(const float* w_oihw, float* w_packed, int cout, int cin, int kh, int kw, void* stream);
int dvg_pack_convT_weight(const float* w_iohw, float* w_packed, int cin, int cout, int kh, int kw, void* stream);
int dvg_unpack_conv_weight(const float* w_packed, float* w_oihw, int cout, int cin, int kh, int kw, void* stream);
int dvg_unpack_convT_weight(const float* w_packed, float* w_iohw, int cin, int cout, int kh, int kw, void* stream);
#define DVG_MODE_CONV3 0
#define DVG_MODE_CONV4S2 1
#define DVG_MODE_CONVT4S2 2
int dvg_conv_first_stats_rows(int ks, int N, int H, int W);
int dvg_mfma_mode(void);
int dvg_packed_row_floats(void);
const char* dvg_build_info(void);
void dvg_set_tile_policy(int energy);
int dvg_tile_policy(void);
int dvg_pack_conv_weight_k16(const float* w, float* w_packed, int cout, int cin, int kh, int kw, int transposed, void* stream);
int dvg_conv_splitk_v2(int mode, int N, int H, int W, int Cin, int Cout);
int dvg_conv_stats_rows_v2(int mode, int N, int H, int W, int Cin, int Cout, int pool, int with_workspace);
int dvg_conv3x3_bn_act_v2(const float* x, const float* skip, const float* w_k16, const float* scale, const float* shift, float* y,
                          float* y_pool, float* stats, int N, int H, int W, int C1, int C2, int Cout, int upsample_x, int act,
                          float slope, float* workspace, long workspace_floats, const float* addend,
                          const int* addend_map, int addend_block, void* stream);
int dvg_conv3x3_first_pair(const float* frame, const float* w0, const float* scale0, const float* shift0, const float* w1_k16,
                           const float* scale1, const float* shift1, float* y, float* y_pool, int N, int H, int W, int Cout, int act, float slope,
                           int y_from , void* stream);
int dvg_pack_conv_weight_wx(const float* w, float* w_packed, int cout, int cin, void* stream);
int dvg_conv3x3_bn_act_wx(const float* x, const float* skip, const float* w_wx, const float* scale, const float* shift, float* y, float* y_pool, int N, int H, int W, int C1, int C2, int Cout, int upsample_x, int act, float slope, const float* addend, const int* addend_map, int addend_block, void* stream);
int dvg_conv3x3_first_pair_wx(const float* frame, const float* w0, const float* scale0, const float* shift0, const float* w1_wx, const float* scale1, const float* shift1, float* y, float* y_pool, int N, int H, int W, int Cout, int act, float slope, int y_from, void* stream);
int dvg_conv4x4s2_bn_act_v2(const float* x, const float* w_k16, const float* scale, const float* shift, float* y, float* stats,
                            int N, int H, int W, int Cin, int Cout, int act, float slope, float* workspace, long workspace_floats, void* stream);
int dvg_convT4x4s2_bn_act_v2(const float* x, const float* skip, const float* w_k16, const float* scale, const float* shift, float* y,
                             float* stats, int N, int H, int W, int C1, int C2, int Cout, int act, float slope, float* workspace,
                             long workspace_floats, const float* addend, const int* addend_map , int addend_block, void* stream);
int dvg_convT4x4s2_bn_act_proj(const float* x, const float* w_k16, const float* scale, const float* shift, const float* proj_w, float* proj_out, int T,
                               int N, int H, int W, int C1, int Cout, int act, float slope, const float* addend, const int* addend_map, int addend_block, void* stream);
int dvg_winograd_weight(const float* w_oihw, float* u_k16, int cout, int cin, int m, void* stream);
int dvg_winograd_input(const float* x, float* v, int N, int H, int W, int C, int m, int upsample, void* stream);
int dvg_gemm_batched_k16(const float* x, const float* w_k16, float* y, int NB, int H, int W, int Cin, int Cout, void* stream);
int dvg_gemm_batched_plan(int NB, int H, int W, int Cin, int Cout, int* tile_w, int* nt, int* ni);
int dvg_winograd_transform_width(long tiles, int C);
int dvg_winograd_output(const float* mm, const float* scale, const float* shift, float* y, float* y_pool, int N, int H, int W, int C, int act, float slope, int m, const float* addend, int y_from , void* stream);
int dvg_winograd_output_input(const float* mm, const float* scale, const float* shift, float* v_next, int N, int H, int W, int C, int act, float slope, const float* addend , void* stream);
int dvg_stem_up_winograd_input(const float* vec, int ldv, const float* w_kn, int KP, const float* scale, const float* shift, float* v_next, int M, int C, int K, int act, float slope, void* stream);
int dvg_winograd_output_up_input(const float* mm, const float* scale, const float* shift, float* v_next, int N, int H, int W, int C, int act, float slope, void* stream);
int dvg_winograd_output_pool_input(const float* m, const float* scale, const float* shift, float* y, float* v_next, int N, int H, int W, int C, int act, float slope, int y_from, void* stream);
int dvg_winograd_input_up_live(const float* x, float* v, int N, int H, int W, int C, void* stream);
int dvg_stem_up_winograd_input_live(const float* vec, int ldv, const float* w_kn, int KP, const float* scale, const float* shift, float* v_next, int M, int C, int K, int act, float slope, void* stream);
int dvg_winograd_output_up_input_live(const float* mm, const float* scale, const float* shift, float* v_next, int N, int H, int W, int C, int act, float slope, void* stream);
int dvg_gemm_batched_k16_as(const float* x, const float* w_k16, float* y, int NB, int NB_as, int H, int W, int Cin, int Cout, void* stream);
int dvg_gemm_batched_plan_as(int NB, int NB_as, int H, int W, int Cin, int Cout, int* tile_w, int* nt, int* ni);
int dvg_winograd_output_input_live(const float* mm, const float* scale, const float* shift, float* v_next, int N, int H, int W, int C, int act, float slope, const float* addend, void* stream);
int dvg_winograd_output_live(const float* mm, const float* scale, const float* shift, float* y, int N, int H, int W, int C, int act, float slope, const float* addend, void* stream);

int dvg_conv3x3_first(const float* x_nchw, const float* w_oihw, const float* scale, const float* shift, float* y, float* stats,
                      int N, int H, int W, int nc, int Cout, int act, float slope, void* stream);

int dvg_convT3x3_last(const float* x, const float* w_iohw, const float* bias, float* y_nchw, int N, int H, int W, int Cin,
                      int nc, int act, void* stream);

int dvg_conv4x4s2_first(const float* x_nchw, const float* w_oihw, const float* scale, const float* shift, float* y, float* stats,
                        int N, int H, int W, int nc, int Cout, int act, float slope, void* stream);

int dvg_convT4x4s2_last(const float* x, const float* skip, const float* w_iohw, const float* bias, float* y_nchw, int N, int H,
                        int W, int C1, int C2, int nc, int act, void* stream);

int dvg_pixel_proj(const float* in, const float* w, float* out, long P, int C, int T, void* stream);

int dvg_convT_gather(const float* d1, const float* d2, const float* bias, float* y_nchw, int ks,
                     int N, int H, int W, int nc, int act,
                     const int* d2_map ,
                     int d2_block, void* stream);


int dvg_channel_stats_rows(long rows);
int dvg_channel_stats(const float* u, float* stats_partial, long rows, int C, int groups, void* stream);
int dvg_channel_stats_pivot(const float* u, float* stats_partial, const float* pivot, long rows, int C, int groups,
                            void* stream);

int dvg_bn_finalize(const float* stats_partial, int nrows, const float* gamma,
                    const float* beta, float* scale, float* shift, float* running_mean,
                    float* running_var, float* save_mean, float* save_invstd,
                    int C, double count, float eps, float momentum,
                    int64_t* num_batches_tracked , int nbt_inc, int groups,
                    float* group_var, void* stream);
int dvg_bn_finalize_pivot(const float* stats_partial, int nrows, const float* pivot, const float* gamma,
                          const float* beta, float* scale, float* shift, float* running_mean, float* running_var,
                          float* save_mean, float* save_invstd, int C, double count, float eps, float momentum,
                          int64_t* num_batches_tracked, int nbt_inc, int groups, float* group_var, void* stream);
int dvg_bn_running_update(const float* mean, const float* unbiased_var, int groups, int C, float mom_first, float mom_mid,
                          float mom_last, float* running_mean, float* running_var, int64_t* num_batches_tracked,
                          int nbt_inc, void* stream);

int dvg_bn_act_apply(const float* u, const float* scale, const float* shift, float* y,
                     float* y_pool, int N, int H, int W, int C, int act, float slope,
                     int group_images, void* stream);

int dvg_gemm_nt_bias_act(const float* a, const float* w, const float* scale, const float* shift, float* out, float* workspace,
                         int M, int N, int K, int lda, int ldo, int period, int splitk, int act, float slope,
                         int accumulate , void* stream);

int dvg_lstm_cell(const float* x, const float* h, const float* c, const float* w_ih, const float* w_hh, const float* b_ih,
                  const float* b_hh, float* h_out, float* c_out, float* gates_out, int B, int H, void* stream);

int dvg_lstm_cell_pre(const float* pre, const float* h, const float* c, const float* w_hh, float* h_out,
                      float* c_out, float* gates_out, int B, int H, void* stream);
int dvg_lstm_cell_bwd(const float* dh_a, const float* dh_b, const float* dc, const float* gates,
                      const float* c_prev, const float* c_new, const float* w_hh_t, float* dG, float* dc_prev,
                      float* dh_prev, int B, int H, void* stream);

int dvg_lstm_cell_x(const float* x, int ldx, int Kx, const float* h, const float* c, const float* w_x, int Kxp,
                    const float* w_hh, const float* bias, float* h_out, float* c_out, int B, int H, void* stream);

int dvg_gru_cell(const float* x, const float* h, const float* w_ih, const float* w_hh, const float* b_ih, const float* b_hh,
                 float* h_out, float* acts_out, int B, int H, void* stream);
int dvg_gru_cell_pre(const float* pre, const float* h, const float* w_hh, const float* b_hn, float* h_out, float* acts_out,
                     int B, int H, void* stream);
int dvg_rnn_cell(const float* x, const float* h, const float* w_ih, const float* w_hh, const float* b_ih, const float* b_hh,
                 float* h_out, int B, int H, void* stream);
int dvg_gru_gates_bwd(const float* dh_a, const float* dh_b, const float* acts, const float* h_prev, float* dGi, float* dGh,
                      float* dh_prev, int B, int H, void* stream);

int dvg_stem_gemm(const float* vec, int ldv, const float* w_kn, int KP, const float* scale, const float* shift,
                  float* out, int ldo, int M, int N, int K, int period, int act, float slope, void* stream);

int dvg_gp_precision(int B, int M, int need_cov);
size_t dvg_gp_lds_bytes(int B, int M, int need_cov);
int dvg_gp_predict(const float* h, const float* z, const float* var_mean, const float* chol_var, const float* mean_const,
                   const float* outputscale, const float* lengthscale, const float* noise, const float* eps, float* mean,
                   float* var, float* sample, float* cov, float* kl, int B, int D, int M, int train_mode, float jitter,
                   int param_period, int step_group, void* stream);
int dvg_gp_step_group(int B, int S, int P, int M);
enum { DVG_GP_KERNEL_RBF = 0, DVG_GP_KERNEL_MATERN12 = 1, DVG_GP_KERNEL_MATERN32 = 2, DVG_GP_KERNEL_MATERN52 = 3 };
int dvg_gp_predict_cov(const float* h, const float* z, const float* var_mean, const float* chol_var, const float* mean_const,
                       const float* outputscale, const float* lengthscale, const float* noise, const float* eps, float* mean,
                       float* var, float* sample, float* cov, float* kl, int B, int D, int M, int train_mode, float jitter,
                       int param_period, int step_group, int cov_kind, void* stream);


int dvg_bn_act_bwd_rows(int N, int H, int W, int pool);
int dvg_bn_act_bwd_reduce(const float* dy, const float* dyp, const float* y, const float* u,
                          float* dp, float* partial, int N, int H, int W, int C, int act,
                          float slope, int groups, void* stream);
int dvg_bn_act_bwd_reduce_centered(const float* dy, const float* dyp, const float* y, const float* u, const float* mean,
                                   float* dp, float* partial, int N, int H, int W, int C, int act, float slope,
                                   int groups, void* stream);
int dvg_bn_bwd_finalize(const float* partial, int nrows, const float* gamma, const float* mean,
                        const float* invstd, float* coefA, float* coefB, float* coefC,
                        float* dgamma, float* dbeta, float* dbias, int C, double count,
                        int train, int accumulate , int groups, void* stream);
int dvg_bn_bwd_finalize_centered(const float* partial, int nrows, const float* gamma, const float* mean,
                                 const float* invstd, float* coefA, float* coefB, float* coefC,
                                 float* dgamma, float* dbeta, float* dbias, int C, double count,
                                 int train, int accumulate, int groups, void* stream);
int dvg_affine3_apply(const float* dp, const float* u, const float* A, const float* B,
                      const float* Cc, float* du, long n, int C, float* sum, int sum_mode,
                      int groups , void* stream);
int dvg_group_sum(const float* src, const int* map, float* dst, int groups, int blocks, long block_elems, void* stream);
int dvg_act_bwd(const float* dy, const float* y, float* dpre, long n, int act, float slope,
                void* stream);
int dvg_upsample2x_bwd(const float* dxu, float* dx, int N, int H, int W, int C, void* stream);
int dvg_colsum(const float* a, float* out, int rows, int C, int accumulate , void* stream);
int dvg_reduce_partials(const float* partial, float* out, int S, long n, void* stream);

int dvg_conv_wgrad_splits(int mode, int N, int H, int W, int Cin, int Cout);
int dvg_conv_wgrad(int mode, const float* x, const float* skip, const float* dout,
                   float* partial, int N, int H, int W, int C1, int C2, int Cout,
                   int upsample_x, void* stream);
int dvg_conv_wgrad_splits_multi(int mode, int N, int H, int W, int Cin, int Cout, int items);
int dvg_conv_wgrad_multi(int mode, int items, const float* const* x, const float* const* skip,
                         const float* const* dout, float* partial, int N, int H, int W, int C1, int C2,
                         int Cout, int upsample_x, void* stream);

int dvg_winograd_wgrad_operands(const float* x, const float* dy, float* v, float* dm, int N, int H, int W, int Cin,
                                int Cout, long t_total, long t_off, void* stream);
int dvg_winograd_wgrad_splits(long t_total, int Cin, int Cout);
int dvg_winograd_wgrad_gemm(const float* dm, const float* v, float* partial, long t_total, int Cin, int Cout, void* stream);
int dvg_winograd_wgrad_gemm_items(const float* dm, const float* const* v_items, int items, long tiles_per_item,
                                  float* partial, int Cin, int Cout, void* stream);
int dvg_winograd_wgrad_reduce(const float* partial, int S, float* packed, int Cin, int Cout, void* stream);

int dvg_wgrad_finish(const float* partial, int S, float* dst, int kind, int kh, int kw, int cout, int cin, int ctot,
                     int c_lo, float beta, void* stream);
int dvg_k4_to_w3(const float* dk4_packed, float* dw, int cout, int c1, int ctot, int c_lo, float beta, void* stream);

int dvg_wgrad_thin_rows(int ks, int N, int Hi, int Wi);
int dvg_wgrad_thin(const float* inp_nchw, const float* dout_nhwc, float* partial, int ks, int N, int Hi, int Wi, int nc, int C, void* stream);

int dvg_moving_mnist_compose(const float* sprites, const int* ids, const int* pos, float* out, int n_sprites, int T, int B, int num_digits, int image_size, int digit_size, void* stream);

int dvg_clip_gather_u8(const uint8_t* pool, const int64_t* first, float* out, int64_t n_frames, int T, int B, int C, int H, int W, int pool_c, void* stream);
int dvg_clip_gather_aug_u8(const uint8_t* pool, const int64_t* first, const int32_t* geom, const float* photo, float* out, int64_t n_frames, int T, int B, int C, int H, int W, int pool_c, void* stream);

int dvg_mnist_scale_u8(const uint8_t* raw, uint8_t* out, int n, int in_size, int out_size, const int* xmin, const int* coef, void* stream);
int dvg_resample_u8_band(const int* ymin_host, int Hin, int Win, int Hout, int Wout, int C, int yk, int* span);
int dvg_resample_u8(const uint8_t* src, uint8_t* dst, int n, int Hin, int Win, int Hout, int Wout, int C, const int* xmin, const int* xcoef, int xk, const int* ymin, const int* ycoef, int yk, const int* ymin_host, void* stream);

int dvg_moving_mnist_compose_u8(const uint8_t* sprites, const int* ids, const int* pos, float* out, int n_sprites, int T, int B, int num_digits, int image_size, int digit_size, void* stream);

int dvg_eval_frames(const float* gt, const float* pred, float* ssim, float* psnr, int n_images, int H, int W,
                    void* stream);

int dvg_eval_frames_finn(const float* gt, const float* pred, float* ssim, float* psnr, float* mse, int n_frames, int C, int H,
                         int W, void* stream);

int dvg_pairwise_frame_mse(const float* samples, float* out, int S, long sample_stride, int frames, long frame_stride, int D,
                           void* stream);

#define DVG_MOSAIC_CELL_INTS 8
#define DVG_MOSAIC_BLACK 0
#define DVG_MOSAIC_RED 1
#define DVG_MOSAIC_GREEN 2
#define DVG_MOSAIC_SEL_NONE 0
#define DVG_MOSAIC_SEL_BEST 1
#define DVG_MOSAIC_SEL_PICK 2
#define DVG_QUANT_TRUNC 0
#define DVG_QUANT_NEAREST 1
int dvg_frame_mosaic(const float* src0, long n0, const float* src1, long n1, const float* src2, long n2, int nc, int H,
                     int W, const int* cells, int F, int R, int Cc, int cell_h, int cell_w, int pad_y, int pad_x, int oy,
                     int ox, const long* best, int n_best, const int* picks, int n_pick_rows, int pick_k,
                     const unsigned char* labels, int n_labels, int lh, int lw, int quant, unsigned char* out,
                     void* stream);

int dvg_adam_step(float* param, const float* grad, float* exp_avg, float* exp_avg_sq, long n, float lr, float beta1,
                  float beta2, float eps, float weight_decay, int step, const int* step_dev, void* stream);

int dvg_gemm_tn(const float* a, const float* b, float* out, float* colsum0, float* colsum1, int R, int M, int N,
                int lda, int ldb, int ldo, int accumulate, int colsum_accumulate, void* stream);
int dvg_lstm_gates_bwd(const float* dh, const float* dc, const float* gates, const float* c_prev, const float* c_new, float* dG,
                       float* dc_prev, int B, int H, void* stream);

int dvg_gp_bwd_precision(int B, int M);
size_t dvg_gp_bwd_lds_bytes(int B, int M);
int dvg_gp_bwd_chunk(int B, int M);
int dvg_gp_train_bwd(const float* h, const float* z, const float* var_mean, const float* chol_var, const float* mean_const,
                     const float* outputscale, const float* lengthscale, const float* gmean, const float* gvar, const float* gkl,
                     float* dh, float* dz, float* dm, float* dls, float* dc, float* ds, float* dell, int B, int D, int M,
                     float jitter, int param_period, int step_group, void* stream);
int dvg_gp_train_bwd_cov(const float* h, const float* z, const float* var_mean, const float* chol_var, const float* mean_const,
                         const float* outputscale, const float* lengthscale, const float* gmean, const float* gvar,
                         const float* gkl, float* dh, float* dz, float* dm, float* dls, float* dc, float* ds, float* dell, int B,
                         int D, int M, float jitter, int param_period, int step_group, int cov_kind, void* stream);
int dvg_sum_steps_multi(const float* const* src, float* const* dst, const long* n, int count, int S, void* stream);

int dvg_gp_elbo(const float* mean, const float* var, const float* kl, const float* target, long t_stride_d,
                long t_stride_b, const float* raw_noise, float* elbo, int B, int D, int num_data,
                int noise_period , void* stream);
int dvg_gp_elbo_bwd(const float* mean, const float* var, const float* kl, const float* target, long t_stride_d, long t_stride_b,
                    const float* raw_noise, const float* gelbo, float* gmean, float* gvar, float* gkl, float* gtarget,
                    float* graw_noise, int B, int D, int num_data, int noise_period, void* stream);

int dvg_nchw_to_nhwc(const float* x, float* y, int N, int C, int H, int W, void* stream);
int dvg_nhwc_to_nchw(const float* x, float* y, int N, int C, int H, int W, void* stream);
void dvg_debug_set_clockbuf(void* buf, unsigned records);
void dvg_debug_set_gp_clockbuf(void* buf, unsigned records);
void dvg_debug_set_wgrad_clockbuf(void* buf, unsigned records);

int dvg_gp_var_norms(const float* var, float* norms, int D, int B, void* stream);
int dvg_gp_trigger_step(const float* var, int D, int B, int col, float* ctx, int window, float coef, int* flag, float* values, float* thresholds, int* flags, int slot, void* stream);
int dvg_gp_trigger_replay(const float* values, int n, const float* ctx0, int window, float coef, int* flags, float* thresholds, void* stream);
int dvg_gp_trigger_select(const int* flag, const float* sample_db, const float* h_pred, float* vec, int D, int B, int n_state, long state_elems, const float* const* state_old, const float* const* state_new, float* const* state_out, void* stream);
int dvg_gp_trigger_rows(const float* var, const float* sample_db, const float* h_pred, float* vec, int D, int B, float* win, int window, int pos, int decide, float coef, int step, int min_gap, int* last, float* values, float* thresholds, int* flags, int slot, void* stream);
int dvg_frame_losses_blocks(long elems);
int dvg_frame_losses(const float* pred, const float* target, float* sums, float* dpred, long n, int S, int K, const float* w,
                     float* partial, void* stream);
int dvg_mse_sum_grad(const float* a, const float* b, float* sum, float* da, long n, float scale, void* stream);
int dvg_frame_losses_ext_blocks(int S, long planes, int H, int W);
int dvg_frame_losses_ext(const float* pred, const float* target, float* sums, float* dpred, int S, int K, long planes, int H, int W,
                         int kind, float eps, const float* w_pix, const float* w_gdl, float* partial, void* stream);
int dvg_frame_ssim_loss_blocks(int S, long planes, int H, int W);
int dvg_frame_ssim_loss(const float* pred, const float* target, float* sums, float* dpred, int S, int K, long planes, int H, int W,
                        const float* w_ssim, int accumulate, double* partial, void* stream);
int dvg_zero_tick(float* g, long n, int* t0, int* t1, int* t2, int* t3, void* stream);
int dvg_grad_sumsq_blocks(long n);
int dvg_grad_sumsq(const float* g, long n, double* partials, void* stream);
int dvg_grad_guard_finish(const double* partials, int nblocks, double max_norm, int skip, float* stat, int* counters, void* stream);
int dvg_adam_step_guarded(float* param, const float* grad, float* exp_avg, float* exp_avg_sq, long n, float lr, float beta1, float beta2,
                          float eps, float weight_decay, int step, const int* step_dev, const float* stat, int* skips_dev, void* stream);
int dvg_lr_schedule_tick(int kind, int W, int N, int K, double R, double G, int* iter_dev, float* scale_dev, void* stream);
int dvg_adam_step_scheduled(float* param, const float* grad, float* exp_avg, float* exp_avg_sq, long n, float lr, float beta1,
                            float beta2, float eps, float weight_decay, int step, const int* step_dev, const float* stat,
                            int* skips_dev, const float* lr_scale_dev, void* stream);
int dvg_optim_step(int rule, float* param, const float* grad, float* m, float* v, long n, float lr, float a, float b, float eps, float weight_decay, int flags,
                   const uint8_t* decay_mask, int step, const int* step_dev, const float* stat, int* skips_dev, const float* lr_scale_dev, void* stream);
int dvg_ema_update_blocks(long n);
int dvg_ema_update(float* ema, const float* param, long n, double decay, const int* updates_dev, double* partials, void* stream);
int dvg_val_accumulate(const float* ssim, const float* psnr, const float* mse, int B, int S, int T, double* acc, long long* cnt,
                       int* best, void* stream);
int dvg_gp_score_slots(int* acc_slots, int* cnt_slots);
int dvg_gp_score(const float* mean, const float* var, const float* noise, int noise_period, const float* target, long t_stride_r, long t_stride_b, int B, int R, double* acc, long long* cnt, void* stream);

#ifdef __cplusplus
}
#endif
#endif
```

Before: 54260.

## Add 2D Winograd F(2x2,3x3) fused 3x3 conv kernel with bf16x3 MFMA

Adds a kernel that applies the Winograd F(2,3) transform in both dimensions to 3x3 convolutions, where the existing WX path transforms only along x. It packs weights into 16 transformed taps, transforms input tiles in LDS each chunk, runs bf16x3 MFMA per tap, and applies the inverse transform in a fused epilogue with BN, activation, pooling and addend. The goal is to cut MFMA work per output from 6 to 4 products per input channel. In exchange it needs larger tiles (8x32), more LDS (one workgroup per CU), W divisible by 32, and adds rounding error from the transforms. The Python wrappers and first-pair dispatch are extended to choose the new form.

```diff
diff --git a/dvg_amd/csrc/conv_igemm2.hip b/dvg_amd/csrc/conv_igemm2.hip
--- a/dvg_amd/csrc/conv_igemm2.hip
+++ b/dvg_amd/csrc/conv_igemm2.hip
@@ -1333,6 +1333,365 @@
     wrow_drain();
 }
 
+#if DVG_BF16X3
+struct CfgWXY {
+    static constexpr int TH = 8, TW = 32, BR = TH / 2, BC = TW / 2, NBLK = BR * BC, HH = TH + 2, HW = TW + 2, HP = HH * HW;
+    static constexpr int LD = 28, LDB = 24, WROW = DVG_WROW;
+    static constexpr int PLANE = NBLK * LD;
+    static constexpr int A_FLOATS = 4 * PLANE, B_FLOATS = 4 * 64 * LDB;
+    static constexpr int NLB = 4 * 64 * WROW / 4 / 256;
+    static constexpr int ND = (HP * 4 + 255) / 256;
+    static constexpr int D_FLOATS = ND * 64 * 16;
+    static constexpr int FP_W = HW + 2, FP_FLOATS = (HH + 2) * FP_W;
+    static constexpr int lds_bytes(bool first) { return (2 * A_FLOATS + 2 * B_FLOATS + 2 * D_FLOATS + (first ? FP_FLOATS : 0)) * 4; }
+    static_assert(NBLK * 4 == 256 && 4 * 64 * WROW / 4 % 256 == 0 && WROW == LDB, "one transform slot per thread, whole passes");
+};
+static_assert(CfgWXY::lds_bytes(true) <= 160 * 1024, "one workgroup per CU");
+
+template <bool FIRST>
+__global__ __launch_bounds__(256, 1) void conv3_wxy_kernel(const Igemm2Params p) {
+    using C = CfgWXY;
+    constexpr int LD = C::LD, LDB = C::LDB, NLB = C::NLB, ND = C::ND;
+    extern __shared__ __attribute__((aligned(16))) float smem[];
+    float* const As = smem;
+    float* const Bs = As + 2 * C::A_FLOATS;
+    float* const Ds = Bs + 2 * C::B_FLOATS;
+    float* const Fp = Ds + 2 * C::D_FLOATS;
+
+    const int tid = threadIdx.x, lane = tid & 63, wave = tid >> 6;
+    const int wm = wave >> 1, wn = wave & 1, l31 = lane & 31, hh = lane >> 5;
+
+    const unsigned lid = xcd_remap(blockIdx.x, gridDim.x);
+    const int tiles_total = p.tiles_x * p.tiles_y * p.tiles_n;
+    const unsigned lr = lid / p.nb_group;
+    const int nb = (int)(lr / tiles_total) * p.nb_group + (int)(lid % p.nb_group);
+    unsigned t = lr % tiles_total;
+    const int tx_i = t % p.tiles_x; t /= p.tiles_x;
+    const int ty_i = t % p.tiles_y; t /= p.tiles_y;
+    const int n0 = (int)t, y0 = ty_i * C::TH, x0 = tx_i * C::TW, yin0 = y0 - 1, xin0 = x0 - 1, nb0 = nb * 64;
+
+    const int a_base = (wm * 32 + l31) * LD + hh * 4;
+    const int b_base = (wn * 32 + l31) * LDB + (hh ^ ((l31 >> 3) & 1)) * 4;
+
+    f32x16 acc[16];
+#pragma unroll
+    for (int f = 0; f < 16; ++f)
+#pragma unroll
+        for (int i = 0; i < 16; ++i) acc[f][i] = 0.f;
+
+    long offx[FIRST ? 1 : ND];
+    unsigned okmask = 0;
+#pragma unroll
+    for (int i = 0; i < ND; ++i) {
+        const int hp = (tid + i * 256) >> 2;
+        const int yy = yin0 + hp / C::HW, xx = xin0 + hp % C::HW;
+        const bool ok = hp < C::HP && (unsigned)yy < (unsigned)p.H && (unsigned)xx < (unsigned)p.W;
+        okmask |= ok ? (1u << i) : 0u;
+        if constexpr (!FIRST) offx[i] = ok ? (((long)n0 * p.H + yy) * p.W + xx) * p.C1 + (tid & 3) * 4 : 0;
+    }
+    const int x_d = ((2 * (tid >> 6)) * C::HW + 2 * ((tid >> 2) & 15)) * 16 + (tid & 3) * 4;
+    const int x_st = (tid >> 2) * LD + (tid & 3) * 2;
+
+    f32x4 fw[FIRST ? 11 : 1];
+    f32x4 ra[ND], rb[NLB];
+    auto gload_d = [&](int c0) {
+        if constexpr (FIRST) {
+            const float* w = p.first_w + c0 + (tid & 3) * 4;
+#pragma unroll
+            for (int tp = 0; tp < 9; ++tp) fw[tp] = *reinterpret_cast<const f32x4*>(w + tp * 64);
+            fw[9] = *reinterpret_cast<const f32x4*>(p.first_scale + c0 + (tid & 3) * 4);
+            fw[10] = *reinterpret_cast<const f32x4*>(p.first_shift + c0 + (tid & 3) * 4);
+        } else {
+            const float* src = p.x + c0;
+#pragma unroll
+            for (int i = 0; i < ND; ++i)
+                ra[i] = *reinterpret_cast<const f32x4*>(((okmask >> i) & 1u) ? src + offx[i] : dvg_zero_slot);
+        }
+    };
+    auto store_d = [&](float* D) {
+        if constexpr (FIRST) {
+#pragma unroll
+            for (int i = 0; i < ND; ++i) {
+                const int hp = min((tid + i * 256) >> 2, C::HP - 1);
+                const float* f = Fp + (hp / C::HW) * C::FP_W + hp % C::HW;
+                f32x4 v = {0.f, 0.f, 0.f, 0.f};
+#pragma unroll
+                for (int tp = 0; tp < 9; ++tp) {
+                    const float px = f[(tp / 3) * C::FP_W + tp % 3];
+#pragma unroll
+                    for (int e = 0; e < 4; ++e) v[e] = fmaf(fw[tp][e], px, v[e]);
+                }
+                const float okf = (float)((okmask >> i) & 1u);
+#pragma unroll
+                for (int e = 0; e < 4; ++e) {
+                    const float a = v[e] * fw[9][e] + fw[10][e];
+                    v[e] = fmaxf(a, a * p.first_slope) * okf;
+                }
+                ra[i] = v;
+            }
+        }
+#pragma unroll
+        for (int i = 0; i < ND; ++i) reinterpret_cast<f32x4*>(D)[tid + i * 256] = ra[i];
+    };
+    auto gload_b = [&](int chunk, int e) {
+        const float* tile = p.w + (((size_t)chunk * (p.Cout >> 6) + nb) * 16 + e * 4) * (64 * C::WROW);
+#pragma unroll
+        for (int j = 0; j < NLB; ++j) rb[j] = reinterpret_cast<const f32x4*>(tile)[tid + j * 256];
+    };
+    auto store_b = [&](float* B) {
+#pragma unroll
+        for (int j = 0; j < NLB; ++j) reinterpret_cast<f32x4*>(B)[tid + j * 256] = rb[j];
+    };
+    auto xform_read = [&](auto e_c, const float* D, u32x2_t (&pa)[4][3]) {
+        constexpr int E = decltype(e_c)::value;
+        constexpr int IA = E == 0 ? 0 : (E == 2 ? 2 : 1), IB = E == 2 ? 1 : (E == 3 ? 3 : 2);
+        f32x4 tj[4], v[4];
+#pragma unroll
+        for (int j = 0; j < 4; ++j) {
+            const f32x4 a = *reinterpret_cast<const f32x4*>(&D[x_d + (IA * C::HW + j) * 16]);
+            const f32x4 b = *reinterpret_cast<const f32x4*>(&D[x_d + (IB * C::HW + j) * 16]);
+#pragma unroll
+            for (int c = 0; c < 4; ++c) tj[j][c] = E == 1 ? a[c] + b[c] : a[c] - b[c];
+        }
+#pragma unroll
+        for (int c = 0; c < 4; ++c) {
+            v[0][c] = tj[0][c] - tj[2][c];
+            v[1][c] = tj[1][c] + tj[2][c];
+            v[2][c] = tj[2][c] - tj[1][c];
+            v[3][c] = tj[1][c] - tj[3][c];
+        }
+#pragma unroll
+        for (int f = 0; f < 4; ++f) {
+            unsigned t0, t1, t2;
+            bf16x3_split_pair(v[f][0], v[f][1], t0, t1, t2);
+            pa[f][0][0] = t0; pa[f][1][0] = t1; pa[f][2][0] = t2;
+            bf16x3_split_pair(v[f][2], v[f][3], t0, t1, t2);
+            pa[f][0][1] = t0; pa[f][1][1] = t1; pa[f][2][1] = t2;
+        }
+    };
+    auto xform_store = [&](float* A, const u32x2_t (&pa)[4][3]) {
+#pragma unroll
+        for (int f = 0; f < 4; ++f)
+#pragma unroll
+            for (int j = 0; j < 3; ++j) *reinterpret_cast<u32x2_t*>(&A[f * C::PLANE + x_st + j * 8]) = pa[f][j];
+    };
+
+    if constexpr (FIRST) {
+        const float* fr = p.first_frame + (size_t)n0 * p.H * p.W;
+        for (int i = tid; i < C::FP_FLOATS; i += 256) {
+            const int yy = yin0 - 1 + i / C::FP_W, xx = xin0 - 1 + i % C::FP_W;
+            Fp[i] = ((unsigned)yy < (unsigned)p.H && (unsigned)xx < (unsigned)p.W) ? fr[(size_t)yy * p.W + xx] : 0.f;
+        }
+        __syncthreads();
+    }
+    gload_d(0);
+    gload_b(0, 0);
+    store_d(Ds);
+    store_b(Bs);
+    gload_b(0, 1);
+    __syncthreads();
+    {
+        u32x2_t pa[4][3];
+        xform_read(std::integral_constant<int, 0>{}, Ds, pa);
+        xform_store(As, pa);
+    }
+    __syncthreads();
+
+    auto stage = [&](const int chunk, auto e_c, auto next_chunk_c, auto has_next_c, auto has_next2_c) __attribute__((always_inline)) {
+        constexpr int E = decltype(e_c)::value, EN = (E + 1) & 3;
+        constexpr bool NEXT_CHUNK = decltype(next_chunk_c)::value, HAS_NEXT = decltype(has_next_c)::value;
+        constexpr bool HAS_NEXT2 = decltype(has_next2_c)::value;
+        constexpr bool LOAD_D = NEXT_CHUNK && E == 0, STORE_D = NEXT_CHUNK && E == 1;
+        const float* const Ac = As + (E & 1) * C::A_FLOATS;
+        const float* const Bc = Bs + (E & 1) * C::B_FLOATS;
+        const int chunk_n = E == 3 ? chunk + 1 : chunk;
+        if constexpr (LOAD_D) gload_d((chunk + 1) * 16);
+        if constexpr (STORE_D) store_d(Ds + ((chunk + 1) & 1) * C::D_FLOATS);
+        f32x4 fa[2][3], fb[2][3];
+#pragma unroll
+        for (int j = 0; j < 3; ++j) {
+            fa[0][j] = *reinterpret_cast<const f32x4*>(&Ac[a_base + j * 8]);
+            fb[0][j] = *reinterpret_cast<const f32x4*>(&Bc[b_base + j * 8]);
+        }
+        u32x2_t pa[4][3];
+        if constexpr (HAS_NEXT) xform_read(std::integral_constant<int, EN>{}, Ds + (chunk_n & 1) * C::D_FLOATS, pa);
+#pragma unroll
+        for (int tt = 0; tt < 4; ++tt) {
+            const int cur = tt & 1, nxt = cur ^ 1;
+            if (tt + 1 < 4) {
+#pragma unroll
+                for (int j = 0; j < 3; ++j) {
+                    fa[nxt][j] = *reinterpret_cast<const f32x4*>(&Ac[a_base + (tt + 1) * C::PLANE + j * 8]);
+                    fb[nxt][j] = *reinterpret_cast<const f32x4*>(&Bc[b_base + (tt + 1) * 64 * LDB + j * 8]);
+                }
+            }
+            if (HAS_NEXT && tt == 3) {
+                xform_store(As + ((E + 1) & 1) * C::A_FLOATS, pa);
+                store_b(Bs + ((E + 1) & 1) * C::B_FLOATS);
+                if constexpr (HAS_NEXT2) gload_b(E >= 2 ? chunk + 1 : chunk, (E + 2) & 3);
+            }
+            auto mm = [&](int pa_, int pb_) {
+                acc[4 * E + tt] = __builtin_amdgcn_mfma_f32_32x32x16_bf16(__builtin_bit_cast(bf16x8_t, fa[cur][pa_]),
+                                                                          __builtin_bit_cast(bf16x8_t, fb[cur][pb_]), acc[4 * E + tt], 0, 0, 0);
+            };
+            mm(2, 0);
+            mm(1, 1);
+            mm(0, 2);
+            mm(1, 0);
+            mm(0, 1);
+            mm(0, 0);
+            constexpr int NREAD = 6, NMFMA = 6;
+            constexpr int NVMEM = LOAD_D ? (FIRST ? 11 : ND) : 0, VPT = (NVMEM + 2) / 3;
+            if (tt == 0) __builtin_amdgcn_sched_group_barrier(0x100, NREAD, 0);
+            if (tt + 1 < 4) {
+#pragma unroll
+                for (int r = 0; r < NREAD; ++r) {
+                    __builtin_amdgcn_sched_group_barrier(0x100, 1, 0);
+                    __builtin_amdgcn_sched_group_barrier(0x008, 1, 0);
+                }
+                if (VPT > 0) __builtin_amdgcn_sched_group_barrier(0x020, VPT, 0);
+            } else if (HAS_NEXT) {
+                constexpr int NW = NLB + 12;
+#pragma unroll
+                for (int r = 0; r < NW; ++r) {
+                    if (r < NMFMA) __builtin_amdgcn_sched_group_barrier(0x008, 1, 0);
+                    __builtin_amdgcn_sched_group_barrier(0x200, 1, 0);
+                }
+            } else {
+                __builtin_amdgcn_sched_group_barrier(0x008, NMFMA, 0);
+            }
+        }
+        if constexpr (HAS_NEXT) __syncthreads();
+    };
+    using std::integral_constant;
+    using T_ = integral_constant<bool, true>;
+    using F_ = integral_constant<bool, false>;
+    const int nchunks = p.C1 / 16;
+    int chunk = 0;
+    for (; chunk + 1 < nchunks; ++chunk) {
+        __builtin_amdgcn_s_setprio(3);
+        stage(chunk, integral_constant<int, 0>{}, T_{}, T_{}, T_{});
+        __builtin_amdgcn_s_setprio(2);
+        stage(chunk, integral_constant<int, 1>{}, T_{}, T_{}, T_{});
+        __builtin_amdgcn_s_setprio(1);
+        stage(chunk, integral_constant<int, 2>{}, T_{}, T_{}, T_{});
+        __builtin_amdgcn_s_setprio(0);
+        stage(chunk, integral_constant<int, 3>{}, T_{}, T_{}, T_{});
+    }
+    stage(chunk, integral_constant<int, 0>{}, F_{}, T_{}, T_{});
+    stage(chunk, integral_constant<int, 1>{}, F_{}, T_{}, T_{});
+    stage(chunk, integral_constant<int, 2>{}, F_{}, T_{}, F_{});
+    stage(chunk, integral_constant<int, 3>{}, F_{}, F_{}, F_{});
+    __builtin_amdgcn_s_setprio(0);
+
+    const int c = nb0 + wn * 32 + l31;
+    const float sc = p.scale ? p.scale[c] : 1.f, sf = p.shift ? p.shift[c] : 0.f;
+    const bool want_y = !FIRST || n0 >= p.y_from;
+    float* const yb = p.y + (size_t)n0 * p.H * p.W * p.Cout + c;
+    float* const pb = p.y_pool ? p.y_pool + (size_t)n0 * (p.H >> 1) * (p.W >> 1) * p.Cout + c : nullptr;
+    const float* ab = nullptr;
+    if (p.addend) ab = p.addend + (size_t)(addend_image(p.add_map, p.add_B, n0)) * p.H * p.W * p.Cout + c;
+    auto epilogue = [&](auto act_c) {
+        constexpr int ACT = decltype(act_c)::value;
+        f32x16 vt[2][2], s1[2];
+#pragma unroll
+        for (int e = 0; e < 4; ++e) {
+            f32x16 s[2];
+#pragma unroll
+            for (int reg = 0; reg < 16; ++reg) {
+                s[0][reg] = (acc[4 * e][reg] + acc[4 * e + 1][reg]) + acc[4 * e + 2][reg];
+                s[1][reg] = (acc[4 * e + 1][reg] - acc[4 * e + 2][reg]) - acc[4 * e + 3][reg];
+            }
+#pragma unroll
+            for (int j = 0; j < 2; ++j)
+#pragma unroll
+                for (int reg = 0; reg < 16; ++reg) {
+                    if (e == 0) vt[0][j][reg] = s[j][reg];
+                    else if (e == 1) { vt[0][j][reg] += s[j][reg]; s1[j][reg] = s[j][reg]; }
+                    else if (e == 2) { vt[0][j][reg] += s[j][reg]; vt[1][j][reg] = s1[j][reg] - s[j][reg]; }
+                    else vt[1][j][reg] -= s[j][reg];
+                }
+            __builtin_amdgcn_sched_barrier(0);
+        }
+#pragma unroll
+        for (int reg = 0; reg < 16; ++reg) {
+            float v[2][2] = {{vt[0][0][reg], vt[0][1][reg]}, {vt[1][0][reg], vt[1][1][reg]}};
+            const int m = wm * 32 + (reg & 3) + 8 * (reg >> 2) + 4 * hh;
+            const int by = (y0 >> 1) + (m >> 4), bx = (x0 >> 1) + (m & 15);
+#pragma unroll
+            for (int i = 0; i < 2; ++i)
+#pragma unroll
+                for (int j = 0; j < 2; ++j) {
+                    const int off = ((2 * by + i) * p.W + 2 * bx + j) * p.Cout;
+                    float u = v[i][j];
+                    if (ab != nullptr) u += ab[off];
+                    u = u * sc + sf;
+                    if constexpr (ACT == DVG_ACT_LRELU) u = u > 0.f ? u : u * p.slope;
+                    else if constexpr (ACT != DVG_ACT_NONE) u = apply_act(u, p.act, p.slope);
+                    v[i][j] = u;
+                    if (want_y) yb[off] = u;
+                }
+            if (pb != nullptr) pb[(by * (p.W >> 1) + bx) * p.Cout] = fmaxf(fmaxf(v[0][0], v[0][1]), fmaxf(v[1][0], v[1][1]));
+        }
+    };
+    if (p.act == DVG_ACT_LRELU) epilogue(std::integral_constant<int, DVG_ACT_LRELU>{});
+    else if (p.act == DVG_ACT_NONE) epilogue(std::integral_constant<int, DVG_ACT_NONE>{});
+    else epilogue(std::integral_constant<int, -1>{});
+}
+
+template <bool FIRST>
+static int launch_wxy(Igemm2Params p, hipStream_t stream) {
+    using C = CfgWXY;
+    p.tiles_y = p.H / C::TH;
+    p.tiles_x = p.W / C::TW;
+    p.tiles_n = p.N;
+    p.nblk_n = p.Cout / 64;
+    const long tiles = (long)p.tiles_y * p.tiles_x * p.tiles_n;
+    p.nb_group = choose_nb_group(tiles, p.nblk_n, 16.0 * p.C1 * 64 * 4, (double)C::TH * C::TW * p.C1 * 4);
+    static bool attr_set = false;
+    if (!attr_set) {
+        hipError_t e = hipFuncSetAttribute(reinterpret_cast<const void*>(&conv3_wxy_kernel<FIRST>),
+                                           hipFuncAttributeMaxDynamicSharedMemorySize, C::lds_bytes(FIRST));
+        if (e != hipSuccess) return fail(DVG_ERR_HIP, "hipFuncSetAttribute: %s", hipGetErrorString(e));
+        attr_set = true;
+    }
+    hipLaunchKernelGGL((conv3_wxy_kernel<FIRST>), dim3((unsigned)(tiles * p.nblk_n)), dim3(256), C::lds_bytes(FIRST), stream, p);
+    return check_launch("conv3_wxy");
+}
+#endif
+
+__global__ void pack_wxy_kernel(const float* __restrict__ src, float* __restrict__ dst, int cout, int cin) {
+    const long total = (long)cout * cin * 16 / 2;
+    const int nblk = cout >> 6;
+    for (long i = blockIdx.x * (long)blockDim.x + threadIdx.x; i < total; i += (long)gridDim.x * blockDim.x) {
+        const int k = (int)(i & 7) * 2;
+        long r = i >> 3;
+        const int co = r % cout; r /= cout;
+        const int tap = r % 16;
+        const int chunk = r / 16;
+        const int e = tap >> 2, f = tap & 3;
+        float u[2];
+#pragma unroll
+        for (int h = 0; h < 2; ++h) {
+            const float* g = src + ((long)co * cin + chunk * 16 + k + h) * 9;
+            float tc[3];
+#pragma unroll
+            for (int cc = 0; cc < 3; ++cc) {
+                if (e == 0) tc[cc] = g[cc];
+                else if (e == 1) tc[cc] = ((g[cc] + g[3 + cc]) + g[6 + cc]) * 0.5f;
+                else if (e == 2) tc[cc] = ((g[cc] - g[3 + cc]) + g[6 + cc]) * 0.5f;
+                else tc[cc] = g[6 + cc];
+            }
+            if (f == 0) u[h] = tc[0];
+            else if (f == 1) u[h] = ((tc[0] + tc[1]) + tc[2]) * 0.5f;
+            else if (f == 2) u[h] = ((tc[0] - tc[1]) + tc[2]) * 0.5f;
+            else u[h] = tc[2];
+        }
+        wrow_store_pair(dst, (((size_t)chunk * nblk + (co >> 6)) * 16 + tap) * 64 + (co & 63), co & 63, k, u[0], u[1]);
+    }
+    wrow_drain();
+}
+
 __global__ void pack_k16_kernel(const float* __restrict__ src, float* __restrict__ dst, int cout, int cin, int kh,
                                 int kw, int transposed) {
     const long total = (long)cout * cin * kh * kw / 2;
@@ -1490,12 +1849,12 @@
     return check_launch("dvg_pack_conv_weight_wx");
 }
 
-static int checks_wx(const Igemm2Params& p, const char* who) {
+static int checks_wx(const Igemm2Params& p, const char* who, int tw = 16) {
     DVG_REQUIRE(p.N > 0 && p.H > 0 && p.W > 0, DVG_ERR_SHAPE, "%s: empty shape", who);
     DVG_REQUIRE(p.C1 > 0 && p.C1 % 16 == 0 && p.C2 == 0 && p.skip == nullptr && !p.upsample, DVG_ERR_SHAPE,
                 "%s: Cin=%d must be a multiple of 16; no concat operand, no upsampling", who, p.C1 + p.C2);
     DVG_REQUIRE(p.Cout > 0 && p.Cout % 64 == 0, DVG_ERR_SHAPE, "%s: Cout=%d must be a multiple of 64", who, p.Cout);
-    DVG_REQUIRE(p.H % 8 == 0 && p.W % 16 == 0, DVG_ERR_SHAPE, "%s: H=%d must be a multiple of 8, W=%d of 16", who, p.H, p.W);
+    DVG_REQUIRE(p.H % 8 == 0 && p.W % tw == 0, DVG_ERR_SHAPE, "%s: H=%d must be a multiple of 8, W=%d of %d", who, p.H, p.W, tw);
     DVG_REQUIRE((long)p.H * p.W * p.Cout < (1L << 31), DVG_ERR_SHAPE, "%s: image of %d x %d x %d floats too large", who, p.H, p.W, p.Cout);
     DVG_REQUIRE(aligned16(p.x) && aligned16(p.w) && aligned16(p.y) && aligned16(p.y_pool) && aligned16(p.addend), DVG_ERR_ALIGN,
                 "%s: pointers must be 16-byte aligned", who);
@@ -1537,6 +1896,54 @@
     if (int e = checks_wx(p, who)) return e;
 #if DVG_BF16X3
     return launch_wx<true>(p, (hipStream_t)stream);
+#else
+    return DVG_ERR_SHAPE;
+#endif
+}
+
+extern "C" int dvg_pack_conv_weight_wxy(const float* w, float* w_packed, int cout, int cin, void* stream) {
+    DVG_REQUIRE(w && w_packed, DVG_ERR_NULL, "dvg_pack_conv_weight_wxy: NULL pointer");
+    DVG_REQUIRE(cout > 0 && cout % 64 == 0 && cin > 0 && cin % 16 == 0, DVG_ERR_SHAPE,
+                "dvg_pack_conv_weight_wxy: Cin must be a multiple of 16, Cout of 64");
+    DVG_REQUIRE(aligned16(w_packed), DVG_ERR_ALIGN, "dvg_pack_conv_weight_wxy: w_packed must be 16-byte aligned");
+    const long total = (long)cout * cin * 16 / 2;
+    hipLaunchKernelGGL(pack_wxy_kernel, dim3(grid_for(total, 256, 4096)), dim3(256), 0, (hipStream_t)stream, w, w_packed, cout, cin);
+    return check_launch("dvg_pack_conv_weight_wxy");
+}
+
+extern "C" int dvg_conv3x3_bn_act_wxy(const float* x, const float* skip, const float* w_wxy, const float* scale,
+                                      const float* shift, float* y, float* y_pool, int N, int H, int W, int C1, int C2,
+                                      int Cout, int upsample_x, int act, float slope, const float* addend,
+                                      const int* addend_map, int addend_block, void* stream) {
+    const char* who = "dvg_conv3x3_bn_act_wxy";
+    DVG_REQUIRE(x && w_wxy && y, DVG_ERR_NULL, "%s: x/w/y must not be NULL", who);
+    Igemm2Params p = params2(x, skip, w_wxy, scale, shift, y, N, H, W, C1, C2, Cout, act, slope);
+    p.y_pool = y_pool;
+    p.upsample = upsample_x ? 1 : 0;
+    if (int e = set_addend(p, who, addend, addend_map, addend_block)) return e;
+    DVG_REQUIRE(addend == nullptr || y_pool == nullptr, DVG_ERR_SHAPE, "%s: addend excludes the pooled output", who);
+    if (int e = checks_wx(p, who, 32)) return e;
+#if DVG_BF16X3
+    return launch_wxy<false>(p, (hipStream_t)stream);
+#else
+    return DVG_ERR_SHAPE;
+#endif
+}
+
+extern "C" int dvg_conv3x3_first_pair_wxy(const float* frame, const float* w0, const float* scale0, const float* shift0,
+                                          const float* w1_wxy, const float* scale1, const float* shift1, float* y, float* y_pool,
+                                          int N, int H, int W, int Cout, int act, float slope, int y_from, void* stream) {
+    const char* who = "dvg_conv3x3_first_pair_wxy";
+    DVG_REQUIRE(frame && w0 && scale0 && shift0 && w1_wxy, DVG_ERR_NULL, "%s: NULL pointer", who);
+    Igemm2Params p;
+    if (int e = first_pair_params(&p, who, frame, w0, scale0, shift0, w1_wxy, scale1, shift1, y, y_pool, N, H, W, Cout, act, slope,
+                                  y_from))
+        return e;
+    DVG_REQUIRE(aligned16(w0) && aligned16(scale0) && aligned16(shift0) && aligned16(y), DVG_ERR_ALIGN,
+                "%s: pointers must be 16-byte aligned", who);
+    if (int e = checks_wx(p, who, 32)) return e;
+#if DVG_BF16X3
+    return launch_wxy<true>(p, (hipStream_t)stream);
 #else
     return DVG_ERR_SHAPE;
 #endif
diff --git a/dvg_amd/fused.py b/dvg_amd/fused.py
--- a/dvg_amd/fused.py
+++ b/dvg_amd/fused.py
@@ -134,12 +134,23 @@
             and ops.wx_workgroups(n, h, w, cout) >= CONV3_WX_MIN_WGS)
 
 
+CONV3_WXY = True
+CONV3_WXY_MIN_WGS = 256
+
+
+def conv3_wxy_applies(n, cin, h, w, cout, *modules) -> bool:
+    return (CONV3_WXY and conv3_wx_applies(n, cin, h, w, cout, *modules) and ops.wxy_ok(n, cin, h, w, cout)
+            and ops.wxy_workgroups(n, h, w, cout) >= CONV3_WXY_MIN_WGS)
+
+
 def _skip_half(kind, skip, ps, conv=None):
     if kind == "conv3" and conv is not None and not conv.training and not torch.is_grad_enabled():
         n, c, h, w = skip.shape
         ctot = conv.weight.shape[1]
         if winograd_tile(n, c, h, w, conv.weight.shape[0]) == 4:
             return ops.conv3x3_winograd(skip, weights.winograd(conv.weight, 4, ctot - c, ctot), None, None, act=ACT_NONE)
+        if conv3_wxy_applies(n, c, h, w, conv.weight.shape[0], conv):
+            return ops.conv3x3_wxy(skip, weights.wxy(conv.weight, ctot - c, ctot), None, None, act=ACT_NONE)
         if conv3_wx_applies(n, c, h, w, conv.weight.shape[0], conv):
             return ops.conv3x3_wx(skip, weights.wx(conv.weight, ctot - c, ctot), None, None, act=ACT_NONE)
     return BLOCKS[kind].raw(skip, None, ps, None)
@@ -448,6 +459,8 @@
             m = winograd_tile(*x.shape, conv.weight.shape[0])
             if m:
                 return _winograd_layer(conv, (sc, sh), x, m, act, slope, pool, y_from, next_conv, next_up)
+            if conv3_wxy_applies(*x.shape, conv.weight.shape[0], conv, bn):
+                return _from(ops.conv3x3_wxy(x, weights.wxy(conv.weight), sc, sh, act=act, slope=slope, pool=pool), y_from)
             if conv3_wx_applies(*x.shape, conv.weight.shape[0], conv, bn):
                 return _from(ops.conv3x3_wx(x, weights.wx(conv.weight), sc, sh, act=act, slope=slope, pool=pool), y_from)
         return _from(ops.conv3x3(x, skip, weights.packed(conv.weight), sc, sh, upsample=upsample, act=act, slope=slope,
@@ -479,6 +492,9 @@
     sc0, sh0 = folded_affine(conv0, bn0)
     sc1, sh1 = folded_affine(conv1, bn1)
     n, _, h, w = x_nchw.shape
+    if conv3_wxy_applies(n, 64, h, w, conv1.out_channels, conv0, bn0, conv1, bn1):
+        return ops.conv3x3_first_pair_wxy(x_nchw, weights.first_pair_taps(conv0.weight), sc0, sh0, weights.wxy(conv1.weight), sc1, sh1,
+                                          slope=slope, pool=pool, y_from=y_from)
     if conv3_wx_applies(n, 64, h, w, conv1.out_channels, conv0, bn0, conv1, bn1):
         return ops.conv3x3_first_pair_wx(x_nchw, weights.first_pair_taps(conv0.weight), sc0, sh0, weights.wx(conv1.weight), sc1, sh1,
                                          slope=slope, pool=pool, y_from=y_from)
diff --git a/dvg_amd/ops/__init__.py b/dvg_amd/ops/__init__.py
--- a/dvg_amd/ops/__init__.py
+++ b/dvg_amd/ops/__init__.py
@@ -5,6 +5,7 @@
 from .conv import (
     pack_conv_weight, pack_convT_weight, packed_row_floats, pack_igemm_weight, _wp_dims, unpack_conv_weight,
     pack_wx_weight, wx_ok, wx_workgroups, conv3x3_wx,
+    pack_wxy_weight, wxy_ok, wxy_workgroups, conv3x3_wxy,
     unpack_convT_weight, _splitk_ws, _SPLITK_WS, evict_captured_workspaces, _stats_buf, _tile_images, SharedBlocks,
     _MAP_CACHE, shared_map, group_sum, _check_addend, conv3x3, CONV4S2_MAX_FLOATS, conv4x4s2, convT4x4s2,
     PROJ_MAX_T, convT4x4s2_proj,
@@ -14,7 +15,7 @@
     conv3x3_winograd, stem_up_winograd_input,
 )
 from .edge import (
-    conv3x3_first, first_pair_ok, conv3x3_first_pair, conv3x3_first_pair_wx, convT3x3_last, conv4x4s2_first, convT4x4s2_last, pixel_proj,
+    conv3x3_first, first_pair_ok, conv3x3_first_pair, conv3x3_first_pair_wx, conv3x3_first_pair_wxy, convT3x3_last, conv4x4s2_first, convT4x4s2_last, pixel_proj,
     _SKIP_PROJ_CACHE, clear_skip_proj_cache, _cached_skip_proj, _last_wmat, _last_wmat_cached,
     precompute_skip_proj, LastProj, convT_last_two_step, eval_frames, eval_frames_finn, pairwise_frame_mse, moving_mnist_compose, clip_gather, clip_gather_aug, CLIP_MAX_SHIFT,
     mnist_scale_u8, moving_mnist_compose_u8, frame_mosaic, QUANT_TRUNC, QUANT_NEAREST,
diff --git a/dvg_amd/ops/conv.py b/dvg_amd/ops/conv.py
--- a/dvg_amd/ops/conv.py
+++ b/dvg_amd/ops/conv.py
@@ -234,6 +234,42 @@
     alg = 2.0 * n * h * w * cout * 9 * cin
     by = 4.0 * (x.numel() + n * h * w * cout + wp.numel())
     _run("conv3x3_igemm", alg * 12 / 18, by, lib().dvg_conv3x3_bn_act_wx, _p(x), None, _p(wp), _p(scale), _p(shift), _p(y),
+         _p(yp), n, h, w, c1, 0, cout, 0, act, slope, _p(addend), _p(amap), ablk, _stream(), alg_flops=alg)
+    return (y, yp) if pool else y
+
+
+def pack_wxy_weight(w: torch.Tensor) -> torch.Tensor:
+    _dev_f32(w, "pack_wxy_weight")
+    w = w.detach().contiguous()
+    co, ci, kh, kw = w.shape
+    if (kh, kw) != (3, 3):
+        raise RuntimeError(f"pack_wxy_weight: a 3x3 kernel is needed, got {kh}x{kw}")
+    out = torch.empty((ci // 16, 16, co, packed_row_floats()), device=w.device, dtype=torch.float32)
+    check(lib().dvg_pack_conv_weight_wxy(_p(w), _p(out), co, ci, _stream()), "pack_wxy")
+    return out
+
+
+def wxy_ok(n, cin, h, w, cout) -> bool:
+    return cin % 16 == 0 and cout % 64 == 0 and h % 8 == 0 and w % 32 == 0 and lib().dvg_mfma_mode() == 1
+
+
+def wxy_workgroups(n, h, w, cout) -> int:
+    return n * (h // 8) * (w // 32) * (cout // 64)
+
+
+def conv3x3_wxy(x, wp, scale, shift, *, act=ACT_LRELU, slope=0.2, pool=False, addend=None):
+    _dev_f32(x, "conv3x3_wxy.x")
+    assert is_nhwc(x), "conv3x3_wxy: x must be NHWC in memory"
+    n, c1, h, w = x.shape
+    taps, cout, cin = _wp_dims(wp)
+    if taps != 16 or cin != c1:
+        raise RuntimeError(f"conv3x3_wxy: packed weight {tuple(wp.shape)} does not match Cin={c1}")
+    y = nhwc_empty(n, cout, h, w, x.device)
+    yp = nhwc_empty(n, cout, h // 2, w // 2, x.device) if pool else None
+    addend, amap, ablk = _check_addend(addend, y, pool)
+    alg = 2.0 * n * h * w * cout * 9 * cin
+    by = 4.0 * (x.numel() + n * h * w * cout + wp.numel())
+    _run("conv3x3_igemm", alg * 8 / 18, by, lib().dvg_conv3x3_bn_act_wxy, _p(x), None, _p(wp), _p(scale), _p(shift), _p(y),
          _p(yp), n, h, w, c1, 0, cout, 0, act, slope, _p(addend), _p(amap), ablk, _stream(), alg_flops=alg)
     return (y, yp) if pool else y
 
diff --git a/dvg_amd/ops/edge.py b/dvg_amd/ops/edge.py
--- a/dvg_amd/ops/edge.py
+++ b/dvg_amd/ops/edge.py
@@ -29,34 +29,46 @@
     return nc == 1 and h % 8 == 0 and w % 16 == 0 and cout % 64 == 0 and n * (h // 8) * (w // 16) * (cout // 64) >= 512
 
 
-def _first_pair(wx, x_nchw, w0, scale0, shift0, w1, scale1, shift1, act, slope, pool, y_from):
-    name, wname = ("conv3x3_first_pair_wx", "wx1") if wx else ("conv3x3_first_pair", "wp1")
+_PAIR_FORMS = {
+    "": ("dvg_conv3x3_first_pair", "wp1", 9, 16, 9),
+    "wx": ("dvg_conv3x3_first_pair_wx", "wx1", 12, 16, 6),
+    "wxy": ("dvg_conv3x3_first_pair_wxy", "wxy1", 16, 32, 4),
+}
+
+
+def _first_pair(form, x_nchw, w0, scale0, shift0, w1, scale1, shift1, act, slope, pool, y_from):
+    entry, wname, want_taps, tw, per_out = _PAIR_FORMS[form]
+    name = entry[4:]
     _dev_f32(x_nchw, name + ".x")
     x = x_nchw if x_nchw.is_contiguous() else x_nchw.contiguous()
     n, nc, h, wd = x.shape
     taps, cout, cin = _wp_dims(w1)
     w0 = w0.detach()
-    ok = h % 8 == 0 and wd % 16 == 0 if wx else first_pair_ok(n, nc, h, wd, cout)
-    if nc != 1 or tuple(w0.shape) != (9, 64) or not w0.is_contiguous() or (taps, cin) != (12 if wx else 9, 64) or not ok:
+    ok = h % 8 == 0 and wd % tw == 0 if form else first_pair_ok(n, nc, h, wd, cout)
+    if nc != 1 or tuple(w0.shape) != (9, 64) or not w0.is_contiguous() or (taps, cin) != (want_taps, 64) or not ok:
         raise RuntimeError(f"{name}: unsupported shapes x {tuple(x.shape)} w0 {tuple(w0.shape)} {wname} {tuple(w1.shape)}")
     if not 0 <= y_from <= n or (y_from and not pool):
         raise RuntimeError(f"{name}: y_from needs the pooled output and 0 <= y_from <= N")
     y = nhwc_empty(n - y_from, cout, h, wd, x.device) if y_from < n else None
     yp = nhwc_empty(n, cout, h // 2, wd // 2, x.device) if pool else None
     alg = 2.0 * n * h * wd * (64 * 9 + cout * 9 * 64)
-    flops = 2.0 * n * h * wd * (64 * 9 + cout * 6 * 64) if wx else alg
+    flops = 2.0 * n * h * wd * (64 * 9 + cout * per_out * 64)
     _run("conv3x3_igemm", flops, 4.0 * (x.numel() + (0 if y is None else y.numel()) + (0 if yp is None else yp.numel()) + w1.numel()),
-         lib().dvg_conv3x3_first_pair_wx if wx else lib().dvg_conv3x3_first_pair, _p(x), _p(w0), _p(scale0), _p(shift0), _p(w1),
+         getattr(lib(), entry), _p(x), _p(w0), _p(scale0), _p(shift0), _p(w1),
          _p(scale1), _p(shift1), _p(y), _p(yp), n, h, wd, cout, act, slope, y_from, _stream(), alg_flops=alg)
     return (y, yp) if pool else y
 
 
 def conv3x3_first_pair(x_nchw, w0, scale0, shift0, wp1, scale1, shift1, *, act=ACT_LRELU, slope=0.2, pool=False, y_from=0):
-    return _first_pair(False, x_nchw, w0, scale0, shift0, wp1, scale1, shift1, act, slope, pool, y_from)
+    return _first_pair("", x_nchw, w0, scale0, shift0, wp1, scale1, shift1, act, slope, pool, y_from)
 
 
 def conv3x3_first_pair_wx(x_nchw, w0, scale0, shift0, wx1, scale1, shift1, *, act=ACT_LRELU, slope=0.2, pool=False, y_from=0):
-    return _first_pair(True, x_nchw, w0, scale0, shift0, wx1, scale1, shift1, act, slope, pool, y_from)
+    return _first_pair("wx", x_nchw, w0, scale0, shift0, wx1, scale1, shift1, act, slope, pool, y_from)
+
+
+def conv3x3_first_pair_wxy(x_nchw, w0, scale0, shift0, wxy1, scale1, shift1, *, act=ACT_LRELU, slope=0.2, pool=False, y_from=0):
+    return _first_pair("wxy", x_nchw, w0, scale0, shift0, wxy1, scale1, shift1, act, slope, pool, y_from)
 
 
 def convT3x3_last(x, w, bias, nc, *, act=ACT_SIGMOID):
diff --git a/dvg_amd/weights.py b/dvg_amd/weights.py
--- a/dvg_amd/weights.py
+++ b/dvg_amd/weights.py
@@ -26,6 +26,11 @@
 def wx(weight, lo=None, hi=None):
     lo, hi, dim = _span(weight, lo, hi, 1)
     return derived(weight, ("wx", lo, hi), (weight,), lambda: ops.pack_wx_weight(_sliced(weight, lo, hi, dim)))
+
+
+def wxy(weight, lo=None, hi=None):
+    lo, hi, dim = _span(weight, lo, hi, 1)
+    return derived(weight, ("wxy", lo, hi), (weight,), lambda: ops.pack_wxy_weight(_sliced(weight, lo, hi, dim)))
 
 
 def split_packed(weight, c1: int, transposed=False):
diff --git a/include/dvg_hip.h b/include/dvg_hip.h
--- a/include/dvg_hip.h
+++ b/include/dvg_hip.h
@@ -46,10 +46,11 @@
 int dvg_pack_conv_weight_wx(const float* w, float* w_packed, int cout, int cin, void* stream);
 int dvg_conv3x3_bn_act_wx(const float* x, const float* skip, const float* w_wx, const float* scale, const float* shift, float* y, float* y_pool, int N, int H, int W, int C1, int C2, int Cout, int upsample_x, int act, float slope, const float* addend, const int* addend_map, int addend_block, void* stream);
 int dvg_conv3x3_first_pair_wx(const float* frame, const float* w0, const float* scale0, const float* shift0, const float* w1_wx, const float* scale1, const float* shift1, float* y, float* y_pool, int N, int H, int W, int Cout, int act, float slope, int y_from, void* stream);
-int dvg_conv4x4s2_bn_act_v2(const float* x, const float* w_k16, const float* scale, const float* shift, float* y, float* stats,
-                            int N, int H, int W, int Cin, int Cout, int act, float slope, float* workspace, long workspace_floats, void* stream);
-int dvg_convT4x4s2_bn_act_v2(const float* x, const float* skip, const float* w_k16, const float* scale, const float* shift, float* y,
-                             float* stats, int N, int H, int W, int C1, int C2, int Cout, int act, float slope, float* workspace,
+int dvg_pack_conv_weight_wxy(const float* w, float* w_packed, int cout, int cin, void* stream);
+int dvg_conv3x3_bn_act_wxy(const float* x, const float* skip, const float* w_wxy, const float* scale, const float* shift, float* y, float* y_pool, int N, int H, int W, int C1, int C2, int Cout, int upsample_x, int act, float slope, const float* addend, const int* addend_map, int addend_block, void* stream);
+int dvg_conv3x3_first_pair_wxy(const float* frame, const float* w0, const float* scale0, const float* shift0, const float* w1_wxy, const float* scale1, const float* shift1, float* y, float* y_pool, int N, int H, int W, int Cout, int act, float slope, int y_from, void* stream);
+int dvg_conv4x4s2_bn_act_v2(const float* x, const float* w_k16, const float* scale, const float* shift, float* y, float* stats, int N, int H, int W, int Cin, int Cout, int act, float slope, float* workspace, long workspace_floats, void* stream);
+int dvg_convT4x4s2_bn_act_v2(const float* x, const float* skip, const float* w_k16, const float* scale, const float* shift, float* y, float* stats, int N, int H, int W, int C1, int C2, int Cout, int act, float slope, float* workspace,
                              long workspace_floats, const float* addend, const int* addend_map , int addend_block, void* stream);
 int dvg_convT4x4s2_bn_act_proj(const float* x, const float* w_k16, const float* scale, const float* shift, const float* proj_w, float* proj_out, int T,
                                int N, int H, int W, int C1, int Cout, int act, float slope, const float* addend, const int* addend_map, int addend_block, void* stream);
```

Measured after the change: 52280. -3.7%, worse.
